# MrTornado24/IDE-3D

Hardware: AMD Instinct MI355X
Metric: 512x512 RGB+seg frames/s @96 depth samples (whole job) (higher is better)
Workload: dtype f32 (3x3 convs + MLPs: fp32 operands as 3 bf16 pieces, 6 products, f32 accumulate); 1 GPU; BASELINE config 2: random-init ide3d-ffhq-64-512, G.mapping + G.synthesis (64 render -> 512, 96 samples, RGB + 19-class seg) + uint8 frames, batch 4 seeds per GPU; global_batch=4, parallelism=dp1, conv_arithmetic=bf16x6, conv_arithmetic_is_library_default=True

## Files before the change

### ide-3d_amd/csrc/modconv.hip

```cpp
#include "common.h"
#include "knobs.h"
#include <stdlib.h>
#include <string.h>
#include <type_traits>

namespace ide3d {

typedef float f32x16 __attribute__((ext_vector_type(16)));

#ifdef IDE3D_MC_TRACE
__device__ unsigned long long g_mc_dbg[256];
#define IDE3D_MC_TS(k) { const unsigned long long now_ = __builtin_readcyclecounter(); mc_acc[k] += now_ - mc_last; mc_last = now_; }
#else
#define IDE3D_MC_TS(k)
#endif

enum { MODE_CONV3 = 0, MODE_CONV1 = 1, MODE_TCONV3 = 2, MODE_TCONV3A = 3, MODE_CONV3S2 = 4 };

template <int MODE> struct ModeCfg;
template <> struct ModeCfg<MODE_CONV3>  { static constexpr int KC = 4, WTAPS = 9, MAXT = 9; };
template <> struct ModeCfg<MODE_CONV1>  { static constexpr int KC = 16, WTAPS = 1, MAXT = 1; };
template <> struct ModeCfg<MODE_CONV3S2> { static constexpr int KC = 4, WTAPS = 9, MAXT = 9; };
template <> struct ModeCfg<MODE_TCONV3> { static constexpr int KC = 4, WTAPS = 9, MAXT = 4; };
template <> struct ModeCfg<MODE_TCONV3A> { static constexpr int KC = 4, WTAPS = 9, MAXT = 9; };

template <int MODE, int BIG, int TI, int PH, int PW>
struct McCfg {
    static constexpr int NWV = 4, NT = 64 * NWV;
    static constexpr int BN = TI * PH * PW;
    static_assert(BN == 64 || BN == 128 || BN == 256, "pixel tile must hold 64, 128 or 256 pixels");
    static constexpr int NCLS = (MODE == MODE_TCONV3A) ? 4 : 1;
    using MC = ModeCfg<MODE>;
    static constexpr int KC = MC::KC, WTAPS = MC::WTAPS, MAXT = MC::MAXT;
    static constexpr int WM = BIG ? 2 : 1, WN = NWV / WM;
    static constexpr int MTW = (BIG == 1) ? 2 : 1;
    static constexpr int NTW = (BN / 32) / WN;
    static constexpr int BM = WM * MTW * 32;
    static constexpr int STRIDE = (MODE == MODE_CONV3S2) ? 2 : 1;
    static constexpr int HALO = (MODE == MODE_CONV1 || MODE == MODE_CONV3S2) ? 0 : 1;
    static constexpr int HP = (MODE == MODE_CONV3S2) ? 2 * PH + 1 : PH + 2 * HALO;
    static constexpr int HW = (MODE == MODE_CONV3S2) ? 2 * PW + 1 : PW + 2 * HALO;
    static constexpr int XW = (MODE == MODE_CONV1) ? PW : (MODE == MODE_CONV3S2) ? ((HW + 3) & ~3) : ((PW == 16) ? 48 : HW + 2);
    static constexpr int XS = HP * XW;
    static constexpr int XI = KC * XS;
    static constexpr int LDS_W = MAXT * KC * BM;
    static constexpr int LDS_X = TI * XI;
    static constexpr int NW4 = (LDS_W / 4 + NT - 1) / NT;
    static constexpr int VW = (MODE == MODE_CONV1 && PH == 1 && PW % 4 == 0) ? 4 : 1;
    static constexpr int NXE = (TI * KC * HP * HW / VW + NT - 1) / NT;
};

template <int N>
__device__ __forceinline__ int sel(const int (&a)[N], int t) {
    int v = a[0];
#pragma unroll
    for (int i = 1; i < N; ++i) v = (t == i) ? a[i] : v;
    return v;
}

__host__ __device__ inline int mc_bm(int cout) { return cout > 96 ? 128 : (cout > 32 ? 64 : 32); }
__host__ __device__ inline int mc_kc(int k) { return k == 3 ? 4 : 16; }

__global__ void __launch_bounds__(256)
modconv_pack_kernel(const float* __restrict__ w, int64_t w_batch_stride, int nbatch, int cout, int cin, int taps, int bm, int kc,
                    int mblocks, int cchunks, float* __restrict__ out) {
    const int64_t total = (int64_t)nbatch * mblocks * cchunks * taps * kc * bm;
    const int64_t stride = (int64_t)gridDim.x * blockDim.x;
    for (int64_t i = (int64_t)blockIdx.x * blockDim.x + threadIdx.x; i < total; i += stride) {
        int64_t r = i;
        const int co_l = (int)(r % bm); r /= bm;
        const int cil = (int)(r % kc); r /= kc;
        const int tap = (int)(r % taps); r /= taps;
        const int cc = (int)(r % cchunks); r /= cchunks;
        const int mb = (int)(r % mblocks); r /= mblocks;
        const int nb = (int)r;
        const int co = mb * bm + co_l, ci = cc * kc + cil;
        out[i] = (co < cout && ci < cin) ? w[nb * w_batch_stride + ((int64_t)co * cin + ci) * taps + tap] : 0.f;
    }
}

struct ConvGeom {
    int tiles_x[4], tiles_y[4];
    int tile_base[5];
    int img_groups;
// ... 436 lines not shown
        const unsigned pk = pk_bf16(a, b);
        out[q] = pk;
        if (q + 1 < PARTS) { a -= __uint_as_float(pk << 16); b -= __uint_as_float(pk & 0xffff0000u); }
    }
    }
}
template <int F16>
__device__ __forceinline__ f32x16 sp_mfma(const u32x4& a, const u32x4& b, const f32x16& c) {
    if constexpr (F16) return __builtin_amdgcn_mfma_f32_32x32x16_f16(__builtin_bit_cast(f16x8, a), __builtin_bit_cast(f16x8, b), c, 0, 0, 0);
    else return __builtin_amdgcn_mfma_f32_32x32x16_bf16(__builtin_bit_cast(bf16x8, a), __builtin_bit_cast(bf16x8, b), c, 0, 0, 0);
}
__device__ __forceinline__ void f16_scale(float bound, float& scale, float& unscale) {
    scale = 1.f; unscale = 1.f;
    if (bound > 0.f && bound < __builtin_inff()) {
        int e;
        frexpf(bound, &e);
        e = min(max(15 - e, -126), 126);
        scale = ldexpf(1.f, e); unscale = ldexpf(1.f, -e);
    }
}

__global__ void __launch_bounds__(256)
modconv_row_scale_kernel(const float* __restrict__ w, int cout, int rowlen, int rows_padded, float* __restrict__ scale, float* __restrict__ unscale) {
    const int row = blockIdx.x * 4 + (threadIdx.x >> 6), lane = threadIdx.x & 63;
    if (row >= rows_padded) return;
    float m = 0.f;
    if (row < cout) for (int i = lane; i < rowlen; i += 64) m = fmaxf(m, fabsf(w[(int64_t)row * rowlen + i]));
#pragma unroll
    for (int off = 32; off > 0; off >>= 1) m = fmaxf(m, __shfl_xor(m, off));
    if (lane == 0) { float sc, us; f16_scale(m, sc, us); scale[row] = sc; unscale[row] = us; }
}

template <int PARTS, int F16 = 0>
__global__ void __launch_bounds__(256)
modconv_pack_split_kernel(const float* __restrict__ w, int cout, int cin, int bm, int mblocks, int cchunks, u32x4* __restrict__ out,
                          const float* __restrict__ row_scale = nullptr) {
    const int64_t total = (int64_t)mblocks * cchunks * 9 * 2 * bm;
    const int64_t stride = (int64_t)gridDim.x * blockDim.x;
    for (int64_t i = (int64_t)blockIdx.x * blockDim.x + threadIdx.x; i < total; i += stride) {
        int64_t r = i;
        const int co_l = (int)(r % bm); r /= bm;
        const int kg = (int)(r % 2); r /= 2;
        const int tap = (int)(r % 9); r /= 9;
        const int cc = (int)(r % cchunks); r /= cchunks;
        const int mb = (int)r;
        const int co = mb * bm + co_l;
        const float rs = F16 ? row_scale[co] : 1.f;
        unsigned pk[4][PARTS];
#pragma unroll
        for (int e = 0; e < 4; ++e) {
            const int ci = cc * 16 + kg * 8 + e * 2;
            const float a = (co < cout && ci < cin) ? w[((int64_t)co * cin + ci) * 9 + tap] * rs : 0.f;
            const float b = (co < cout && ci + 1 < cin) ? w[((int64_t)co * cin + ci + 1) * 9 + tap] * rs : 0.f;
            split_pair<PARTS, F16>(a, b, pk[e]);
        }
        const int64_t base = (((int64_t)(mb * cchunks + cc) * 9 + tap) * PARTS * 2 + kg) * bm + co_l;
#pragma unroll
        for (int q = 0; q < PARTS; ++q) {
            const u32x4 v = {pk[0][q], pk[1][q], pk[2][q], pk[3][q]};
            out[base + (int64_t)q * 2 * bm] = v;
        }
    }
}

template <int OFF_BYTES>
__device__ __forceinline__ u32x4 lds_read128_async(unsigned addr) {
    u32x4 v;
    asm volatile("ds_read_b128 %0, %1 offset:%2" : "=v"(v) : "v"(addr), "n"(OFF_BYTES));
    return v;
}
template <int PENDING>
__device__ __forceinline__ void lds_wait128(u32x4& first) { asm volatile("s_waitcnt lgkmcnt(%1)" : "+v"(first) : "n"(PENDING)); }
__device__ __forceinline__ void lds_pin128(u32x4& v) { asm volatile("" : "+v"(v)); }

struct HeadEpi {
    const u32x4* w;
    const float* bias;
    float* y;
    int rows;
    float clamp;
    int store_x;
    int bias_first;
};
template <int PH, int PW, int NWV, int MTW, int NTW, int BM, int MT, int PARTS, int SCRATCH>
__device__ __forceinline__ void split_heads_finish(const ide3d_modconv_params& p, const HeadEpi& he, f32x16 (&acc)[1][MTW][NTW], float* smem,
                                                   int n0, int y0, int x0, int wm, int wn, int lp) {
    constexpr int NT = 64 * NWV, BN = PH * PW, TP = BN + 4, ROWS = MT * 32, CCH = BM / 16, A_UNITS = PARTS * 2 * ROWS;
    static_assert(BM * TP + 2 * BM + ROWS <= SCRATCH, "activation tile + coefficients must fit the loop's LDS");
    const int tid = threadIdx.x, lane = tid & 63, half = lane >> 5, l32 = lane & 31;
    const int wid = __builtin_amdgcn_readfirstlane(tid >> 6);
    const int hw = p.h * p.w_;
    float* const s_t = smem;
    float* const s_dm = smem + BM * TP;
    float* const s_bi = s_dm + BM;
    float* const s_hb = s_bi + BM;
    for (int e = tid; e < BM; e += NT) {
        s_dm[e] = (p.dcoefs && e < p.cout) ? p.dcoefs[(int64_t)n0 * p.cout + e] : 1.f;
        s_bi[e] = (p.bias && e < p.cout) ? p.bias[e] : 0.f;
    }
    for (int e = tid; e < ROWS; e += NT) s_hb[e] = (he.bias && e < he.rows) ? he.bias[e] : 0.f;
    __syncthreads();
    const float e_alpha = (p.act == 3) ? p.alpha : 1.f, e_gain = p.gain;
    const float e_clamp = (p.clamp >= 0.f) ? p.clamp : __builtin_inff();
    const float e_nstr = p.noise ? p.noise_strength : 0.f;
    auto finish = [&](float v, float d, float nz, float bb) {
        v *= d; v += nz; v += bb;
        v = (v > 0.f) ? v : v * e_alpha;
        v *= e_gain;
        return fminf(fmaxf(v, -e_clamp), e_clamp);
    };
#pragma unroll
    for (int j = 0; j < NTW; ++j) {
        const int pix = (wn * NTW + j) * 32 + lp;
        const int gy = y0 + pix / PW, gx = x0 + pix % PW;
        const float nz = (e_nstr != 0.f) ? p.noise[gy * p.w_ + gx] * e_nstr : 0.f;
#pragma unroll
        for (int i = 0; i < MTW; ++i)
#pragma unroll
            for (int r = 0; r < 16; ++r) {
                const int rl = (wm * MTW + i) * 32 + (r & 3) + 8 * (r >> 2) + 4 * half;
                s_t[rl * TP + pix] = finish(acc[0][i][j][r], s_dm[rl], nz, s_bi[rl]);
            }
    }
    __syncthreads();
    typedef float f32x4a __attribute__((ext_vector_type(4)));
    typedef float f32x4u __attribute__((ext_vector_type(4), aligned(4)));
    if (he.store_x) {
        float* const yimg = p.y + (int64_t)n0 * p.cout * hw;
#pragma unroll 4
        for (int e = tid; e < BM * BN / 4; e += NT) {
            const int rl = e / (BN / 4), pix = (e % (BN / 4)) * 4;
            const int gy = y0 + pix / PW, gx = x0 + pix % PW;
            *reinterpret_cast<f32x4u*>(yimg + (int64_t)rl * hw + gy * p.w_ + gx) = *reinterpret_cast<const f32x4a*>(s_t + rl * TP + pix);
        }
    }
    constexpr int NPT = BN / 32;
    constexpr int RG = (MT % 2 == 0 && NPT / NWV < 2) ? 2 : 1, MTH = MT / RG, PG = NWV / RG, NTH = NPT / PG;
    static_assert(MTH * RG == MT && NTH * PG == NPT && NTH >= 1, "head work must split evenly over the waves");
    const int rg = wid / PG, pg = wid % PG;
    const u32x4* __restrict__ wsrc = he.w + (int64_t)n0 * CCH * A_UNITS + half * ROWS + rg * MTH * 32 + l32;
    f32x16 hacc[MTH][NTH];
#pragma unroll
    for (int m = 0; m < MTH; ++m)
#pragma unroll
        for (int g = 0; g < 4; ++g) {
            const f32x4a b4 = *reinterpret_cast<const f32x4a*>(s_hb + (rg * MTH + m) * 32 + 8 * g + 4 * half);
#pragma unroll
            for (int t = 0; t < NTH; ++t)
#pragma unroll
                for (int k = 0; k < 4; ++k) hacc[m][t][4 * g + k] = he.bias_first ? b4[k] : 0.f;
        }
    u32x4 af[2][MTH][PARTS];
    auto fetch_a = [&](int c, int buf) {
#pragma unroll
        for (int m = 0; m < MTH; ++m)
#pragma unroll
            for (int q = 0; q < PARTS; ++q) af[buf][m][q] = wsrc[(int64_t)c * A_UNITS + q * 2 * ROWS + m * 32];
    };
    fetch_a(0, 0);
#pragma unroll
    for (int c = 0; c < CCH; ++c) {
        const int ab = c & 1;
        if (c + 1 < CCH) fetch_a(c + 1, ab ^ 1);
#pragma unroll
        for (int t = 0; t < NTH; ++t) {
            const float* xs = s_t + (c * 16 + 8 * half) * TP + (pg * NTH + t) * 32 + l32;
            u32x4 bfrag[PARTS];
            {
                unsigned pk[4][PARTS];
#pragma unroll
                for (int e = 0; e < 4; ++e) split_pair<PARTS>(xs[(2 * e) * TP], xs[(2 * e + 1) * TP], pk[e]);
#pragma unroll
                for (int q = 0; q < PARTS; ++q) bfrag[q] = u32x4{pk[0][q], pk[1][q], pk[2][q], pk[3][q]};
            }
#pragma unroll
            for (int m = 0; m < MTH; ++m)
#pragma unroll
                for (int qa = 0; qa < PARTS; ++qa)
#pragma unroll
                    for (int qb = 0; qa + qb < PARTS; ++qb)
                        hacc[m][t] = __builtin_amdgcn_mfma_f32_32x32x16_bf16(__builtin_bit_cast(bf16x8, af[ab][m][qa]), __builtin_bit_cast(bf16x8, bfrag[qb]), hacc[m][t], 0, 0, 0);
        }
    }
    const float h_clamp = (he.clamp >= 0.f) ? he.clamp : __builtin_inff();
#pragma unroll
    for (int t = 0; t < NTH; ++t) {
        const int pix = (pg * NTH + t) * 32 + l32;
        const int gy = y0 + pix / PW, gx = x0 + pix % PW;
        float* const o = he.y + (int64_t)n0 * he.rows * hw + gy * p.w_ + gx;
#pragma unroll
        for (int m = 0; m < MTH; ++m)
#pragma unroll
            for (int r = 0; r < 16; ++r) {
                const int row = (rg * MTH + m) * 32 + 8 * (r >> 2) + 4 * half + (r & 3);
                if (row >= he.rows) continue;
                float v = hacc[m][t][r];
                if (he.bias_first) {
                    v = __builtin_amdgcn_fmed3f(v, -h_clamp, h_clamp);
                } else {
                    v *= 1.f; v += 0.f; v += s_hb[row];
                    v = (v > 0.f) ? v : v * 1.f;
                    v = fminf(fmaxf(v, -h_clamp), h_clamp);
                }
                o[(int64_t)row * hw] = v;
            }
    }
    __syncthreads();
}

template <int MODE, int BIG, int PH, int PARTS, int WBUF, int NWV, int F16, int TEAMS = 1, int PAR = -1, int HEAD_MT = 0>
__device__ __forceinline__ void modconv_split_tile(const ide3d_modconv_params& p, const u32x4* __restrict__ wp, float* __restrict__ partial,
                                                   const ConvGeom& g, unsigned char* smem, int mb, int tl, int grp, int split, int tiles_x,
                                                   const float* __restrict__ row_unscale, float* wg_scratch = nullptr, const HeadEpi* he = nullptr) {
    using K = SpCfg<MODE, BIG, PH, PARTS, WBUF, NWV, (PAR >= 0)>;
    static_assert(!F16 || PARTS == 2, "f16x3 = two fp16 pieces per operand");
    static_assert(PAR < 0 || (MODE == MODE_TCONV3A && WBUF == 2 && TEAMS == 1), "row-parity pairs: transposed form, two weight buffers, one team");
    constexpr int NST = (PAR < 0) ? 3 : (PAR == 0 ? 2 : 1);
    auto kys = [](int i) constexpr { return (PAR < 0) ? i : (PAR == 0 ? 2 * i : 1); };
    static_assert(TEAMS == 1 || (TEAMS == 2 && NWV == 4), "two teams of four waves, or one team");
    constexpr int PW = K::PW;
    const int tid = (TEAMS == 2) ? (int)(threadIdx.x & 255u) : (int)threadIdx.x, lane = tid & 63;
    const int wid = __builtin_amdgcn_readfirstlane(tid >> 6);
    const int wm = wid / K::WN, wn = wid % K::WN;
    const int half = lane >> 5, l32 = lane & 31;
    const int lp = ((((l32 >> 2) ^ (l32 >> 3) ^ (l32 >> 4)) & 1) << 4) | (l32 & 15);
    const int txi = tl % tiles_x, tyi = tl / tiles_x;
    const int y0 = tyi * PH, x0 = txi * PW;
    const int n0 = grp;
    u32x4* const s_w = reinterpret_cast<u32x4*>(smem);
    u32x4* const s_x = s_w + WBUF * K::W_UNITS;

    f32x16 acc[K::NCLS][K::MTW][K::NTW];
#pragma unroll
    for (int q = 0; q < K::NCLS; ++q)
#pragma unroll
        for (int i = 0; i < K::MTW; ++i)
#pragma unroll
            for (int j = 0; j < K::NTW; ++j)
#pragma unroll
                for (int r = 0; r < 16; ++r) acc[q][i][j][r] = 0.f;

    const int hw = p.h * p.w_;
    int x_src[K::NXR];
#pragma unroll
    for (int r = 0; r < K::NXR; ++r) {
        const int sidx = lane + 64 * r;
        const int ry = sidx / K::HW, rx = sidx % K::HW;
        const int yy = y0 - 1 + ry, xx = x0 - 1 + rx;
        x_src[r] = (sidx < K::NSLOT && yy >= 0 && yy < p.h && xx >= 0 && xx < p.w_) ? yy * p.w_ + xx : -1;
    }
    const float* __restrict__ ximg = p.x + (int64_t)n0 * p.cin * hw;
    float xreg[K::NXR][4];
    float sty[4];
    float xs = 1.f, xus = 1.f;
    if constexpr (F16) {
        float mm = p.styles ? 0.f : 1.f;
        if (p.styles) for (int ci = lane; ci < p.cin; ci += 64) mm = fmaxf(mm, fabsf(p.styles[(int64_t)n0 * p.cin + ci]));
        float xm = (lane < IDE3D_AMAX_SLOTS) ? p.x_amax[(int64_t)n0 * IDE3D_AMAX_FLOATS + lane * IDE3D_AMAX_STRIDE] : 0.f;
#pragma unroll
        for (int off = 32; off > 0; off >>= 1) { mm = fmaxf(mm, __shfl_xor(mm, off)); xm = fmaxf(xm, __shfl_xor(xm, off)); }
        f16_scale(mm * xm, xs, xus);
    }
    const bool stages_patch = (NWV == 4) || wid < 4;
    auto fetch_patch = [&](int c) {
        if (!stages_patch) return;
        const int ci0 = c * K::KC + wid * 4;
#pragma unroll
        for (int k = 0; k < 4; ++k) {
            const int ci = min(ci0 + k, p.cin - 1);
            sty[k] = (ci0 + k < p.cin) ? (p.styles ? p.styles[(int64_t)n0 * p.cin + ci] : 1.f) : 0.f;
#pragma unroll
            for (int r = 0; r < K::NXR; ++r) xreg[r][k] = ximg[(int64_t)ci * hw + max(x_src[r], 0)];
        }
    };
    auto commit_patch = [&](int buf) {
        if (!stages_patch) return;
        unsigned char* const dst = reinterpret_cast<unsigned char*>(s_x + buf * K::X_UNITS) + ((wid >> 1) * K::NSLOT) * 16 + (wid & 1) * 8;
        const float sc[4] = {F16 ? sty[0] * xs : sty[0], F16 ? sty[1] * xs : sty[1], F16 ? sty[2] * xs : sty[2], F16 ? sty[3] * xs : sty[3]};
#pragma unroll
        for (int r = 0; r < K::NXR; ++r) {
            const int sidx = lane + 64 * r;
            const bool live = x_src[r] >= 0;
            unsigned lo[PARTS], hi[PARTS];
            split_pair<PARTS, F16>(live ? xreg[r][0] * sc[0] : 0.f, live ? xreg[r][1] * sc[1] : 0.f, lo);
            split_pair<PARTS, F16>(live ? xreg[r][2] * sc[2] : 0.f, live ? xreg[r][3] * sc[3] : 0.f, hi);
            if (sidx < K::NSLOT) {
#pragma unroll
                for (int q = 0; q < PARTS; ++q) {
                    const u32x2 v = {lo[q], hi[q]};
                    *reinterpret_cast<u32x2*>(dst + (q * 2 * K::NSLOT + sidx) * 16) = v;
                }
            }
        }
    };
    const u32x4* __restrict__ wsrc = wp + (int64_t)mb * g.cchunks * 3 * K::W_UNITS;
    constexpr int W_PIECES = K::W_UNITS / 64;
// ... 44 lines not shown
        const bool more = c + 1 < c_end;
        static_for<NST>([&](auto sii) {
            constexpr int SI = decltype(sii)::value, KY = kys(SI);
            constexpr bool LAST = (SI == NST - 1), MID = (SI == (NST == 3 ? 1 : 0));
            const int next_stage = LAST ? (c + 1) * 3 + kys(0) : c * 3 + kys(LAST ? 0 : SI + 1);
            IDE3D_MC_TS(0)
            if constexpr (WBUF == 2) {
                if (!LAST || more) fetch_weights(next_stage, wbuf ^ 1);
                if (MID && more) fetch_patch(c + 1);
            } else {
                fetch_weights(c * 3 + KY, 0);
                if (MID && more) fetch_patch(c + 1);
                asm volatile("s_waitcnt vmcnt(0)" ::: "memory");
                __syncthreads();
            }
            IDE3D_MC_TS(1)
            const unsigned a_base = a_base0 + ((WBUF == 2) ? wbuf * (K::W_UNITS * 16) : 0);
            unsigned b_base[K::NTW];
#pragma unroll
            for (int j = 0; j < K::NTW; ++j) b_base[j] = b_base0[j] + xbuf * (K::X_UNITS * 16);
            constexpr int GRP = K::MTW + K::NTW, NGRP = 3 * PARTS;
            constexpr int SP_AHEAD = 1;
            constexpr int NBUF = (PARTS == 2 && SP_AHEAD > 1) ? 3 : 2;
            constexpr int AHEAD_CAP = 15 / GRP - 1, AHEAD_SAFE = (NBUF - 1) * PARTS - 1;
            constexpr int AHEAD = (SP_AHEAD < AHEAD_CAP ? SP_AHEAD : AHEAD_CAP) < AHEAD_SAFE ? (SP_AHEAD < AHEAD_CAP ? SP_AHEAD : AHEAD_CAP) : AHEAD_SAFE;
            static_assert(AHEAD >= 1 && (AHEAD + 1) * GRP <= 15, "lgkmcnt is a 4-bit counter");
            constexpr bool B_REUSE = (MODE == MODE_TCONV3A) && NBUF == 2;
            u32x4 av[NBUF][K::MTW][PARTS], bv[NBUF][K::NTW][PARTS];
            auto issue = [&](auto ss) {
                constexpr int S = decltype(ss)::value, KX = S / PARTS, Q = S % PARTS, B = KX % NBUF, T = KY * 3 + KX;
                constexpr int BS = B_REUSE ? (KX == 2 ? 1 : 0) : B;
                static_for<K::MTW>([&](auto ii) {
                    constexpr int I = decltype(ii)::value;
                    av[B][I][Q] = lds_read128_async<(((KX * PARTS + Q) * 2) * K::BM + I * 32) * 16>(a_base);
                });
                if constexpr (!(B_REUSE && KX == 1))
                static_for<K::NTW>([&](auto jj) {
                    constexpr int J = decltype(jj)::value;
                    bv[BS][J][Q] = lds_read128_async<(Q * 2 * K::NSLOT + tap_patch_offset<MODE, K::HW>(T)) * 16>(b_base[J]);
                });
            };
            static_for<AHEAD>([&](auto ss) { issue(ss); });
            static_for<NGRP>([&](auto ss) {
                constexpr int S = decltype(ss)::value, KX = S / PARTS, Q = S % PARTS, B = KX % NBUF, QC = (PAR >= 0) ? (KX & 1) : tap_class<MODE>(KY * 3 + KX);
                constexpr int BS = B_REUSE ? (KX == 2 ? 1 : 0) : B;
                if constexpr (S + AHEAD < NGRP) issue(std::integral_constant<int, S + AHEAD>{});
                constexpr int PENDING = [] { int n = 0; for (int s2 = S + 1; s2 <= S + AHEAD && s2 < NGRP; ++s2) n += K::MTW + ((B_REUSE && s2 / PARTS == 1) ? 0 : K::NTW); return n; }();
                lds_wait128<PENDING>(av[B][0][Q]);
#pragma unroll
                for (int i = 0; i < K::MTW; ++i) lds_pin128(av[B][i][Q]);
                if constexpr (!(B_REUSE && KX == 1)) {
#pragma unroll
                for (int j = 0; j < K::NTW; ++j) lds_pin128(bv[BS][j][Q]);
                }
#pragma unroll
                for (int qa = 0; qa <= Q; ++qa)
#pragma unroll
                    for (int qb = 0; qb <= Q; ++qb) {
                        if ((qa == Q || qb == Q) && qa + qb < PARTS) {
#pragma unroll
                            for (int i = 0; i < K::MTW; ++i)
#pragma unroll
                                for (int j = 0; j < K::NTW; ++j)
                                    acc[QC][i][j] = sp_mfma<F16>(av[B][i][qa], bv[BS][j][qb], acc[QC][i][j]);
                        }
                    }
            });
            IDE3D_MC_TS(2)
            if (LAST && more) commit_patch(xbuf ^ 1);
            if constexpr (WBUF == 2 && NWV == 8) { if (!LAST || more) fetch_weights(next_stage, wbuf ^ 1, true); }
            IDE3D_MC_TS(3)
            if (WBUF == 2) asm volatile("s_waitcnt vmcnt(0)" ::: "memory");
            IDE3D_MC_TS(4)
            __syncthreads();
            IDE3D_MC_TS(5)
            wbuf ^= 1;
        });
    }
#ifdef IDE3D_MC_TRACE
    const unsigned long long mc_t1 = __builtin_readcyclecounter();
#endif
    if constexpr (HEAD_MT > 0) {
        static_assert(MODE == MODE_CONV3 && TEAMS == 1 && !F16 && K::NCLS == 1, "fused heads: 3x3 split-bf16 layers");
        split_heads_finish<PH, PW, K::NWV, K::MTW, K::NTW, K::BM, HEAD_MT, PARTS, K::LDS_BYTES / 4>(p, *he, acc, reinterpret_cast<float*>(smem), n0, y0, x0, wm, wn, lp);
    } else
    modconv_finish<MODE, 1, PH, PW, K::NWV, K::NCLS, K::MTW, K::NTW, K::BM, K::LDS_BYTES / 4, PAR>(p, partial, g, acc, reinterpret_cast<float*>(smem), mb, n0, y0, x0, split, 0, wm, wn, lp,
                                                                                                F16 ? row_unscale : nullptr, xus, (TEAMS == 2) ? tid : -1, wg_scratch);
#ifdef IDE3D_MC_TRACE
    if (blockIdx.x == 100 && (threadIdx.x == 0 || threadIdx.x == 256)) {
        const int o = threadIdx.x ? 16 : 0;
        for (int k = 0; k < 6; ++k) g_mc_dbg[o + k] = mc_acc[k];
        g_mc_dbg[o + 7] = (unsigned long long)(c_end - c_begin) * 3;
        g_mc_dbg[o + 8] = mc_prologue;
        g_mc_dbg[o + 9] = __builtin_readcyclecounter() - mc_t1;
    }
#endif
}



constexpr int head_waves(int mt) { return mt == 1 ? 16 : 8; }
template <int PARTS, int MT>
struct HeadCfg {
    static constexpr int ROWS = MT * 32;
    static constexpr int A_UNITS = PARTS * 2 * ROWS;
    static constexpr int NWV = head_waves(MT);
    static constexpr int BN = 32 * NWV;
};
__host__ __device__ inline int64_t head_packed_units(int n, int cchunks, int parts, int mt) { return (int64_t)n * cchunks * parts * 2 * mt * 32; }

template <int PARTS>
__global__ void __launch_bounds__(256)
head_pack_split_kernel(const float* __restrict__ w, int64_t w_batch_stride, int n, int cout, int cin, int rows, int cchunks, u32x4* __restrict__ out) {
    const int64_t total = (int64_t)n * cchunks * 2 * rows;
    const int64_t stride = (int64_t)gridDim.x * blockDim.x;
    for (int64_t i = (int64_t)blockIdx.x * blockDim.x + threadIdx.x; i < total; i += stride) {
        int64_t r = i;
        const int row = (int)(r % rows); r /= rows;
        const int kg = (int)(r % 2); r /= 2;
        const int cc = (int)(r % cchunks); r /= cchunks;
        const int nb = (int)r;
        unsigned pk[4][PARTS];
#pragma unroll
        for (int e = 0; e < 4; ++e) {
            const int ci = cc * 16 + kg * 8 + e * 2;
            const float a = (row < cout && ci < cin) ? w[nb * w_batch_stride + (int64_t)row * cin + ci] : 0.f;
            const float b = (row < cout && ci + 1 < cin) ? w[nb * w_batch_stride + (int64_t)row * cin + ci + 1] : 0.f;
            split_pair<PARTS>(a, b, pk[e]);
        }
        const int64_t base = (((int64_t)nb * cchunks + cc) * PARTS * 2 + kg) * rows + row;
#pragma unroll
        for (int q = 0; q < PARTS; ++q) {
            const u32x4 v = {pk[0][q], pk[1][q], pk[2][q], pk[3][q]};
            out[base + (int64_t)q * 2 * rows] = v;
        }
    }
}

template <int PARTS, int MT>
__global__ void __launch_bounds__(64 * head_waves(MT), head_waves(MT) / 4)
head_split_kernel(ide3d_modconv_params p, const u32x4* __restrict__ wp, int cchunks, int tiles_per_image) {
    using K = HeadCfg<PARTS, MT>;
    if constexpr (K::NWV == 16) asm volatile("" ::: "v127"); else asm volatile("" ::: "v255");
    constexpr int S_MIN = K::NWV * 32 * 40 / 4 + 2 * K::ROWS / 4 + 16;
    constexpr int S_UNITS = (2 * K::A_UNITS > S_MIN) ? 2 * K::A_UNITS : S_MIN;
    __shared__ __attribute__((aligned(16))) u32x4 s_a[S_UNITS];
    const int tid = threadIdx.x, lane = tid & 63, half = lane >> 5, l32 = lane & 31;
    const int wid = __builtin_amdgcn_readfirstlane(tid >> 6);
    const int bid = xcd_remap(blockIdx.x, gridDim.x);
    const int n0 = bid / tiles_per_image, tile = bid % tiles_per_image;
    const int hw = p.h * p.w_;
    const int pix = tile * K::BN + wid * 32 + l32;
    const int pix_c = min(pix, hw - 1);
    const float* __restrict__ xl = p.x + (int64_t)n0 * p.cin * hw + (int64_t)(8 * half) * hw + pix_c;
    const u32x4* __restrict__ wsrc = wp + (int64_t)n0 * cchunks * K::A_UNITS;

    f32x16 acc[1][MT][1];
#pragma unroll
    for (int m = 0; m < MT; ++m)
#pragma unroll
        for (int r = 0; r < 16; ++r) acc[0][m][0][r] = 0.f;

    constexpr int A_PIECES = K::A_UNITS / 64;
    static_assert(K::A_UNITS % 64 == 0, "whole 1 KB pieces");
    auto fetch_a = [&](int c, int buf) {
        for (int i = wid; i < A_PIECES; i += K::NWV)
            __builtin_amdgcn_global_load_lds((const __attribute__((address_space(1))) void*)(wsrc + (int64_t)c * K::A_UNITS + i * 64 + lane),
// ... 321 lines not shown
                const float vb = ok_b ? xb[k] * scv[k] : 0.f;
                const float4 a0 = wv[0], a1 = wv[1], c0v = wv[4], c1v = wv[5];
                const float w0[STRIP_CO] = {a0.x, a0.y, a0.z, a0.w, a1.x, a1.y, a1.z, a1.w};
                const float w2[STRIP_CO] = {c0v.x, c0v.y, c0v.z, c0v.w, c1v.x, c1v.y, c1v.z, c1v.w};
#pragma unroll
                for (int j = 0; j < STRIP_CO; ++j) { acc[j] = fmaf(va, w0[j], acc[j]); acc[j] = fmaf(vb, w2[j], acc[j]); }
            }
        }
    }
#pragma unroll
    for (int j = 0; j < STRIP_CO; ++j) s_red[q][j][lane] = acc[j];
    __syncthreads();
    float am = 0.f;
    {
        static_assert(STRIP_CO <= STRIP_WAVES, "wave q < STRIP_CO finishes output channel co0 + q");
        float v = 0.f;
        const int qc = min(q, STRIP_CO - 1);
#pragma unroll
        for (int k = 0; k < STRIP_WAVES; ++k) v += s_red[k][qc][lane];
        const int co = co0 + q;
        if (live && q < STRIP_CO && co < p.cout) {
            v *= p.dcoefs ? p.dcoefs[(int64_t)n * p.cout + co] : 1.f;
            const int oy = is_row ? oh - 1 : t, ox = is_row ? t : ow - 1;
            p.y[((int64_t)n * p.cout + co) * ((int64_t)oh * pitch) + (int64_t)oy * pitch + ox] = v;
            amax_acc(am, v);
        }
    }
    if (p.y_amax) amax_raise_block(p.y_amax, n, am, s_am);
}

struct BlockId { int mb, tile, grp, split; };
__device__ __forceinline__ BlockId decode_block(const ConvGeom& g) {
    int bid = xcd_remap(blockIdx.x, gridDim.x);
    BlockId b;
    b.mb = bid % g.mblocks; bid /= g.mblocks;
    b.tile = bid % g.tile_base[4]; bid /= g.tile_base[4];
    b.grp = bid % g.img_groups; bid /= g.img_groups;
    b.split = bid;
    return b;
}

template <int MODE, int BIG, int TI, int PH, int PW>
__global__ void __launch_bounds__(256, (McCfg<MODE, BIG, TI, PH, PW>::NCLS * McCfg<MODE, BIG, TI, PH, PW>::MTW * McCfg<MODE, BIG, TI, PH, PW>::NTW > 8) ? 1
                                       : (TI * PH * PW <= 128 && MODE != MODE_CONV3S2) ? 3 : 2)
modconv_kernel(ide3d_modconv_params p, const float* __restrict__ wp, float* __restrict__ partial, ConvGeom g) {
    using K = McCfg<MODE, BIG, TI, PH, PW>;
    __shared__ __attribute__((aligned(16))) float s_w[2 * K::LDS_W];
    __shared__ __attribute__((aligned(16))) float s_x[2 * K::LDS_X];
    const BlockId b = decode_block(g);
    int cls = 0;
    if (MODE == MODE_TCONV3) { cls = (b.tile >= g.tile_base[1]) + (b.tile >= g.tile_base[2]) + (b.tile >= g.tile_base[3]); }
    modconv_tile<MODE, BIG, TI, PH, PW>(p, wp, partial, g, s_w, s_x, b.mb, b.tile - g.tile_base[cls], b.grp, b.split, cls, g.tiles_x[cls]);
}


#ifdef IDE3D_SP_SHARED_SIMD
constexpr bool kSpExclusive = false;
#else
constexpr bool kSpExclusive = true;
#endif
template <int MODE, int BIG, int PH, int PARTS, int WBUF, int NWV>
constexpr int sp_waves_per_simd() {
    using K = SpCfg<MODE, BIG, PH, PARTS, WBUF, NWV>;
    return (NWV == 8) ? 2 : (!kSpExclusive && K::LDS_BYTES <= 80 * 1024 && (WBUF == 1 || K::NCLS * K::MTW * K::NTW <= 8)) ? 2 : 1;
}
template <int MODE, int BIG, int PH, int PARTS, int WBUF = 2, int NWV = 4, int F16 = 0>
__global__ void __launch_bounds__(64 * NWV, (sp_waves_per_simd<MODE, BIG, PH, PARTS, WBUF, NWV>()))
modconv_split_kernel(ide3d_modconv_params p, const u32x4* __restrict__ wp, float* __restrict__ partial, ConvGeom g, const float* __restrict__ row_unscale) {
    using K = SpCfg<MODE, BIG, PH, PARTS, WBUF, NWV>;
    if constexpr (kSpExclusive) { if constexpr (NWV == 8) asm volatile("" ::: "v255"); else asm volatile("" ::: "v255", "a255"); }
    __shared__ __attribute__((aligned(16))) unsigned char sp_smem[K::LDS_BYTES];
    const BlockId b = decode_block(g);
    modconv_split_tile<MODE, BIG, PH, PARTS, WBUF, NWV, F16>(p, wp, partial, g, sp_smem, b.mb, b.tile, b.grp, b.split, g.tiles_x[0], row_unscale);
}

template <int BIG, int PH, int HEAD_MT>
__global__ void __launch_bounds__(512, 2)
modconv_split_heads_kernel(ide3d_modconv_params p, const u32x4* __restrict__ wp, ConvGeom g, HeadEpi he) {
    using K = SpCfg<MODE_CONV3, BIG, PH, 3, 2, 8>;
    if constexpr (kSpExclusive) asm volatile("" ::: "v255");
    __shared__ __attribute__((aligned(16))) unsigned char sp_smem[K::LDS_BYTES];
    const BlockId b = decode_block(g);
    modconv_split_tile<MODE_CONV3, BIG, PH, 3, 2, 8, 0, 1, -1, HEAD_MT>(p, wp, nullptr, g, sp_smem, b.mb, b.tile, b.grp, b.split, g.tiles_x[0], nullptr, nullptr, &he);
}

template <int BIG, int PH, int PARTS, int F16 = 0>
__global__ void __launch_bounds__(512, 2)
modconv_split_pair_kernel(ide3d_modconv_params p, const u32x4* __restrict__ wp, float* __restrict__ partial, ConvGeom g, const float* __restrict__ row_unscale) {
    using K = SpCfg<MODE_TCONV3A, BIG, PH, PARTS, 2, 8, 1>;
    if constexpr (kSpExclusive) asm volatile("" ::: "v255");
    __shared__ __attribute__((aligned(16))) unsigned char sp_smem[K::LDS_BYTES];
    const int half_grid = (int)(gridDim.x >> 1);
    const int par = __builtin_amdgcn_readfirstlane((int)blockIdx.x >= half_grid ? 1 : 0);
    int bid = xcd_remap((int)blockIdx.x - par * half_grid, half_grid);
    BlockId b;
    b.mb = bid % g.mblocks; bid /= g.mblocks;
    b.tile = bid % g.tile_base[4]; bid /= g.tile_base[4];
    b.grp = bid % g.img_groups; bid /= g.img_groups;
    b.split = bid;
    if (par == 0) modconv_split_tile<MODE_TCONV3A, BIG, PH, PARTS, 2, 8, F16, 1, 0>(p, wp, partial, g, sp_smem, b.mb, b.tile, b.grp, b.split, g.tiles_x[0], row_unscale);
    else          modconv_split_tile<MODE_TCONV3A, BIG, PH, PARTS, 2, 8, F16, 1, 1>(p, wp, partial, g, sp_smem, b.mb, b.tile, b.grp, b.split, g.tiles_x[0], row_unscale);
}

template <int MODE, int BIG, int PH, int PARTS, int WBUF, int F16>
__global__ void __launch_bounds__(512, 2)
modconv_split_teams_kernel(ide3d_modconv_params p, const u32x4* __restrict__ wp, float* __restrict__ partial, ConvGeom g, const float* __restrict__ row_unscale) {
    using K = SpCfg<MODE, BIG, PH, PARTS, WBUF, 4>;
    static_assert(2 * K::LDS_BYTES <= 160 * 1024, "both teams' LDS must fit");
    asm volatile("" ::: "v255");
    __shared__ __attribute__((aligned(16))) unsigned char sp_smem[2 * K::LDS_BYTES];
    const int team = (int)(threadIdx.x >> 8);
    int bid = xcd_remap(blockIdx.x, gridDim.x);
    const int mpairs = g.mblocks >> 1;
    BlockId b;
    b.mb = 2 * (bid % mpairs) + team; bid /= mpairs;
    b.tile = bid % g.tile_base[4]; bid /= g.tile_base[4];
    b.grp = bid % g.img_groups; bid /= g.img_groups;
    b.split = bid;
    modconv_split_tile<MODE, BIG, PH, PARTS, WBUF, 4, F16, 2>(p, wp, partial, g, sp_smem + team * K::LDS_BYTES, b.mb, b.tile, b.grp, b.split, g.tiles_x[0], row_unscale,
                                                              reinterpret_cast<float*>(sp_smem));
}

__global__ void __launch_bounds__(256)
modconv_epilogue_kernel(ide3d_modconv_params p, const float* __restrict__ partial, int split_k, int oh, int ow) {
    const int64_t per = (int64_t)p.n * p.cout * oh * ow;
    const int64_t stride = (int64_t)gridDim.x * blockDim.x;
    int am_n = -1; float am = 0.f;
    __shared__ unsigned s_am[64];
    const bool am_lds = p.y_amax && p.n <= 64;
    if (p.y_amax) { if (threadIdx.x < 64) s_am[threadIdx.x] = 0u; __syncthreads(); }
    const int hw = oh * ow;
    if (p.y_pitch <= 0 && (hw & 3) == 0) {
        typedef float f32x4v __attribute__((ext_vector_type(4)));
        const int64_t per4 = per >> 2;
        for (int64_t q = (int64_t)blockIdx.x * blockDim.x + threadIdx.x; q < per4; q += stride) {
            const int64_t i = q << 2;
            f32x4v v = {0.f, 0.f, 0.f, 0.f};
            int s = 0;
            for (; s + 4 <= split_k; s += 4) {
                f32x4v t[4];
#pragma unroll
                for (int k = 0; k < 4; ++k) t[k] = *reinterpret_cast<const f32x4v*>(partial + (int64_t)(s + k) * per + i);
#pragma unroll
                for (int k = 0; k < 4; ++k) v += t[k];
            }
            for (; s < split_k; ++s) v += *reinterpret_cast<const f32x4v*>(partial + (int64_t)s * per + i);
            const int pix = (int)(i % hw);
            const int co = (int)((i / hw) % p.cout);
            const int n = (int)(i / ((int64_t)hw * p.cout));
            const float d = p.dcoefs ? p.dcoefs[(int64_t)n * p.cout + co] : 1.f, bb = p.bias ? p.bias[co] : 0.f;
#pragma unroll
            for (int e = 0; e < 4; ++e) {
                float x = v[e];
                if (p.dcoefs) x *= d;
                if (p.noise) x += p.noise[pix + e] * p.noise_strength;
                if (p.bias) x += bb;
                if (p.act == 3) x = (x > 0.f) ? x : x * p.alpha;
                x *= p.gain;
                if (p.clamp >= 0.f) x = fminf(fmaxf(x, -p.clamp), p.clamp);
                v[e] = x;
            }
            *reinterpret_cast<f32x4v*>(p.y + i) = v;
            if (p.y_amax) {
                if (n != am_n) { if (am_n >= 0) { if (am_lds) amax_lds_flush(s_am, am_n, am); else amax_commit(p.y_amax, am_n, am, false); } am_n = n; am = 0.f; }
                amax_acc(am, v[0]); amax_acc(am, v[1]); amax_acc(am, v[2]); amax_acc(am, v[3]);
            }
// ... 361 lines not shown
    IDE3D_CHECK_ARG(p.act == 1 || p.act == 3, "modconv2d: act must be linear (1) or lrelu (3)");
    IDE3D_CHECK_ARG(p.y_pitch == 0 || (p.mode == 2 && p.y_pitch >= 2 * p.w_ + 1), "modconv2d: y_pitch is the row pitch of a transposed convolution's output (>= 2 w + 1), or 0");
    hipStream_t st_head = (hipStream_t)stream;
    {
        const int64_t hw = (int64_t)p.h * p.w_;
        if (head_small_applies(p)) {
            if (hw <= 64) hipLaunchKernelGGL((head_small_kernel<64, 32>), dim3(cdiv(p.cout, HS_RB), 1, p.n), dim3(HS_THREADS), 0, st_head, p, (int)hw);
            else          hipLaunchKernelGGL((head_small_kernel<256, 8>), dim3(cdiv(p.cout, HS_RB), cdiv((int)hw, 256), p.n), dim3(HS_THREADS), 0, st_head, p, (int)hw);
            IDE3D_CHECK_LAUNCH("modconv2d (small-map heads)");
            return IDE3D_OK;
        }
    }
    if (head_split_applies(p, resolve_arith(p.arith))) {
        const int parts = resolve_arith(p.arith) == 3 ? 2 : 3, mt = p.cout <= 32 ? 1 : 6, cchunks = cdiv(p.cin, 16);
        IDE3D_CHECK_ARG(p.workspace_bytes >= head_packed_units(p.n, cchunks, parts, mt) * 16, "modconv2d: workspace too small for the packed head weights");
        u32x4* wu = reinterpret_cast<u32x4*>(p.workspace);
        const int64_t items = (int64_t)p.n * cchunks * 2 * mt * 32;
        const int tiles = cdiv(p.h * p.w_, 32 * head_waves(mt));
        const int hw_h = p.h * p.w_, wgs_img = kNumCU / p.n, tiles32 = hw_h / 32;
        const bool resident = head_resident_applies(p);
#define IDE3D_HEAD_RES(P, M, C) IDE3D_EXCL_LAUNCH((head_resident_kernel<P, M, C>), dim3(p.n * wgs_img), 512, 0, st_head, p, wu, wgs_img, tiles32)
#define IDE3D_HEAD(P, M) do { \
            hipLaunchKernelGGL(head_pack_split_kernel<P>, dim3(stream_grid(items, 256)), dim3(256), 0, st_head, p.w, p.w_batch_stride, p.n, p.cout, p.cin, M * 32, cchunks, wu); \
            if (resident) { if (M == 6) IDE3D_HEAD_RES(P, 6, 8); else if (cchunks == 4) IDE3D_HEAD_RES(P, 1, 4); else IDE3D_HEAD_RES(P, 1, 8); } \
            else IDE3D_EXCL_LAUNCH((head_split_kernel<P, M>), dim3(p.n * tiles), 64 * head_waves(M), 0, st_head, p, wu, cchunks, tiles); } while (0)
        if (parts == 2) { if (mt == 1) IDE3D_HEAD(2, 1); else IDE3D_HEAD(2, 6); }
        else            { if (mt == 1) IDE3D_HEAD(3, 1); else IDE3D_HEAD(3, 6); }
#undef IDE3D_HEAD
#undef IDE3D_HEAD_RES
        IDE3D_CHECK_LAUNCH("modconv2d (split-bf16 heads)");
        return IDE3D_OK;
    }
    int arith_eff = resolve_arith(p.arith);
    if (arith_eff == 16 && !p.x_amax) arith_eff = 6;
    ConvPlan pl; plan_conv(p, pl, arith_eff);
    IDE3D_CHECK_ARG(p.workspace_bytes >= (pl.packed_floats + pl.aux_floats + pl.partial_floats) * (int64_t)sizeof(float),
                    "modconv2d: workspace too small (need %lld bytes)", (long long)((pl.packed_floats + pl.aux_floats + pl.partial_floats) * sizeof(float)));
    hipStream_t st = (hipStream_t)stream;
    float* wp = p.workspace;
    float* partial = p.workspace + pl.packed_floats + pl.aux_floats;
    if (pl.parts) {
        if (!p.weights_packed) pack_split_weights(p, pl, wp, st);
#define IDE3D_SP_DISPATCH(M) \
        do { if (pl.big == 1) { if (pl.f16) launch_split<M, 1, 2, 1>(p, pl, wp, partial, st); else if (pl.parts == 2) launch_split<M, 1, 2>(p, pl, wp, partial, st); else launch_split<M, 1, 3>(p, pl, wp, partial, st); } \
             else             { if (pl.f16) launch_split<M, 2, 2, 1>(p, pl, wp, partial, st); else if (pl.parts == 2) launch_split<M, 2, 2>(p, pl, wp, partial, st); else launch_split<M, 2, 3>(p, pl, wp, partial, st); } } while (0)
        if (pl.mode == MODE_CONV3) IDE3D_SP_DISPATCH(MODE_CONV3); else IDE3D_SP_DISPATCH(MODE_TCONV3A);
#undef IDE3D_SP_DISPATCH
    } else {
    if (!p.weights_packed) {
        hipLaunchKernelGGL(modconv_pack_kernel, dim3(stream_grid(pl.packed_floats, 256)), dim3(256), 0, st,
                           p.w, p.w_batch_stride, p.w_batch_stride ? p.n : 1, p.cout, p.cin, pl.taps, pl.bm, pl.kc, pl.mblocks, pl.cchunks, wp);
    }
#define IDE3D_MC_DISPATCH(M) \
    do { if (pl.big == 1) launch_tiles<M, 1>(p, pl, wp, partial, st); else if (pl.big == 2) launch_tiles<M, 2>(p, pl, wp, partial, st); \
         else launch_tiles<M, 0>(p, pl, wp, partial, st); } while (0)
    if (pl.mode == MODE_CONV3)       IDE3D_MC_DISPATCH(MODE_CONV3);
    else if (pl.mode == MODE_CONV1)  IDE3D_MC_DISPATCH(MODE_CONV1);
    else if (pl.mode == MODE_CONV3S2) IDE3D_MC_DISPATCH(MODE_CONV3S2);
    else if (pl.mode == MODE_TCONV3A) IDE3D_MC_DISPATCH(MODE_TCONV3A);
    else                             IDE3D_MC_DISPATCH(MODE_TCONV3);
#undef IDE3D_MC_DISPATCH
    }
    if (pl.g.split_k > 1) {
        const int64_t per = (int64_t)p.n * p.cout * pl.oh * pl.ow;
        hipLaunchKernelGGL(modconv_epilogue_kernel, dim3(stream_grid((p.y_pitch <= 0 && ((pl.oh * pl.ow) & 3) == 0) ? per / 4 : per, 256)), dim3(256), 0, st, p, partial, pl.g.split_k, pl.oh, pl.ow);
    }
    if (pl.mode == MODE_TCONV3A && !p.weights_packed) {
        hipLaunchKernelGGL(tconv_strip_pack_kernel, dim3(stream_grid(pl.strip_floats, 256)), dim3(256), 0, st, p.w, p.cout, p.cin, cdiv(p.cout, STRIP_CO) * STRIP_CO,
                           wp + pl.packed_floats + pl.strip_off);
    }
    if (pl.strip) {
        const int cout_pad = cdiv(p.cout, STRIP_CO) * STRIP_CO;
        float* const wstrip = wp + pl.packed_floats + pl.strip_off;
        const int nb_re = cdiv(p.w_ + 1, 64), nb_ro = cdiv(p.w_, 64), nb_ce = cdiv(p.h, 64), nb_co = cdiv(p.h, 64);
        float* const xs = wstrip + pl.strip_floats;
        hipLaunchKernelGGL(tconv_strip_gather_kernel, dim3(stream_grid((int64_t)p.n * p.cin * (p.h + p.w_), 256)), dim3(256), 0, st, p.x, p.n * p.cin, p.h, p.w_, xs);
        hipLaunchKernelGGL(tconv_strip_kernel, dim3(nb_re + nb_ro + nb_ce + nb_co, cout_pad / STRIP_CO, p.n), dim3(64 * STRIP_WAVES), 0, st, p, wstrip, xs, cout_pad,
                           pl.oh, pl.ow, (int64_t)(p.y_pitch > 0 ? p.y_pitch : pl.ow), nb_re, nb_ro, nb_ce);
    }
    IDE3D_CHECK_LAUNCH("modconv2d");
    return IDE3D_OK;
}

extern "C" int ide3d_modconv2d_heads(const ide3d_modconv_params* pp, const ide3d_modconv_head_epilogue* hp, void* stream) {
    using namespace ide3d;
    IDE3D_CHECK_ARG(pp != nullptr && hp != nullptr, "modconv2d_heads: null params");
    const ide3d_modconv_params& p = *pp;
    const ide3d_modconv_head_epilogue& h = *hp;
    IDE3D_CHECK_ARG(p.x && p.w && p.workspace && (p.y || h.no_activation_output) && h.w && h.y && h.workspace, "modconv2d_heads: null tensor / workspace pointer");
    int rc = check_modconv(p);
    if (rc) return rc;
    IDE3D_CHECK_ARG(p.act == 1 || p.act == 3, "modconv2d_heads: act must be linear (1) or lrelu (3)");
    IDE3D_CHECK_ARG(h.rows > 0, "modconv2d_heads: bad head rows");
    auto no_kernel = [](const char* why) { set_error("modconv2d_heads: %s", why); return IDE3D_ENOKERNEL; };
    if (knob_live("IDE3D_MODCONV_NO_HEAD_FUSION")) return no_kernel("IDE3D_MODCONV_NO_HEAD_FUSION is set");
    if (p.k != 3 || p.mode != 0 || p.w_batch_stride != 0 || p.y_amax || p.y_pitch != 0) return no_kernel("not a shared-weight 3x3 layer without side outputs");
    int arith = resolve_arith(p.arith);
    if (arith == 16 && !p.x_amax) arith = 6;
    if (arith != 6) return no_kernel("the fused form exists for bf16x6 only");
    ConvPlan pl; plan_conv(p, pl, arith);
    if (pl.parts != 3 || pl.f16 || pl.mode != MODE_CONV3 || pl.pair || pl.g.split_k != 1 || pl.g.mblocks != 1 || pl.bm != p.cout || kTiles[pl.tile].images != 1)
        return no_kernel("the layer's plan does not hold all channels of a tile in one workgroup");
    const bool tile16 = pl.big == 1 && p.cout == 128 && pl.tile == T16x16 && sp_form(pl).waves == 8;
    const bool tile32 = pl.big == 2 && p.cout == 64 && pl.tile == T32x16;
    const int ph = tile32 ? 32 : 16;
    if (!(tile16 || tile32) || p.h % ph != 0 || p.w_ % 16 != 0) return no_kernel("no fused instance for this tile");
    ide3d_modconv_params q{};
    q.x = p.y; q.w = h.w; q.bias = h.bias; q.y = h.y;
    q.n = p.n; q.cin = p.cout; q.cout = h.rows; q.h = p.h; q.w_ = p.w_; q.k = 1; q.mode = 0;
    q.act = 1; q.alpha = 0.f; q.gain = 1.f; q.clamp = h.clamp; q.w_batch_stride = (int64_t)h.rows * p.cout; q.arith = p.arith;
    const int mt = h.rows <= 32 ? 1 : 6, hcc = p.cout / 16;
    if (head_small_applies(q) || !head_split_applies(q, resolve_arith(q.arith)) || resolve_arith(q.arith) == 3 || (mt == 6 && !tile16))
        return no_kernel("the heads do not take the split-bf16 path");
    IDE3D_CHECK_ARG(p.workspace_bytes >= (pl.packed_floats + pl.aux_floats) * (int64_t)sizeof(float), "modconv2d_heads: workspace too small");
    IDE3D_CHECK_ARG(h.workspace_bytes >= head_packed_units(p.n, hcc, 3, mt) * 16, "modconv2d_heads: head workspace too small");
    hipStream_t st = (hipStream_t)stream;
    if (!p.weights_packed) pack_split_weights(p, pl, p.workspace, st);
    u32x4* const hw_packed = reinterpret_cast<u32x4*>(h.workspace);
    const int64_t items = (int64_t)p.n * hcc * 2 * mt * 32;
    hipLaunchKernelGGL(head_pack_split_kernel<3>, dim3(stream_grid(items, 256)), dim3(256), 0, st, h.w, q.w_batch_stride, p.n, h.rows, p.cout, mt * 32, hcc, hw_packed);
    HeadEpi e;
    e.w = hw_packed; e.bias = h.bias; e.y = h.y; e.rows = h.rows; e.clamp = h.clamp; e.store_x = !h.no_activation_output;
    e.bias_first = head_resident_applies(q) ? 1 : 0;
    const ConvGeom& g = pl.g;
    const unsigned nblocks = (unsigned)((int64_t)g.mblocks * g.tile_base[4] * g.img_groups * g.split_k);
    const u32x4* wu = reinterpret_cast<const u32x4*>(p.workspace);
    if (tile32) IDE3D_EXCL_LAUNCH((modconv_split_heads_kernel<2, 32, 1>), dim3(nblocks), 512, 0, st, p, wu, g, e);
    else if (mt == 1) IDE3D_EXCL_LAUNCH((modconv_split_heads_kernel<1, 16, 1>), dim3(nblocks), 512, 0, st, p, wu, g, e);
    else IDE3D_EXCL_LAUNCH((modconv_split_heads_kernel<1, 16, 6>), dim3(nblocks), 512, 0, st, p, wu, g, e);
    IDE3D_CHECK_LAUNCH("modconv2d_heads");
    return IDE3D_OK;
}

extern "C" int ide3d_modconv_plan(const ide3d_modconv_params* pp, ide3d_modconv_plan_info* out) {
    using namespace ide3d;
    IDE3D_CHECK_ARG(pp != nullptr && out != nullptr, "modconv_plan: null argument");
    const ide3d_modconv_params p = flatten_pointwise(*pp);
    int rc = check_modconv(p);
    if (rc) return rc;
    *out = ide3d_modconv_plan_info{};
    const int arith = resolve_arith(p.arith);
    if (head_small_applies(p)) {
        const int hw = p.h * p.w_;
        out->kind = IDE3D_PLAN_HEAD_SMALL; out->tile_h = 1; out->tile_w = hw <= 64 ? 64 : 256; out->rows = HS_RB; out->waves = HS_THREADS / 64; out->split_k = 1;
        out->workgroups = (int64_t)cdiv(p.cout, HS_RB) * (hw <= 64 ? 1 : cdiv(hw, 256)) * p.n;
        return IDE3D_OK;
    }
    if (head_split_applies(p, arith)) {
        const int mt = p.cout <= 32 ? 1 : 6;
        out->rows = mt * 32; out->parts = arith == 3 ? 2 : 3; out->split_k = 1; out->tile_h = 1;
        if (head_resident_applies(p)) { out->kind = IDE3D_PLAN_HEAD_RESIDENT; out->tile_w = 32; out->waves = 8; out->workgroups = (int64_t)p.n * (kNumCU / p.n); }
        else { out->kind = IDE3D_PLAN_HEAD_SPLIT; out->waves = head_waves(mt); out->tile_w = 32 * out->waves; out->workgroups = (int64_t)p.n * cdiv(p.h * p.w_, out->tile_w); }
        return IDE3D_OK;
    }
    int arith_eff = arith;
    if (arith_eff == 16 && !p.x_amax) arith_eff = 6;
    ConvPlan pl; plan_conv(p, pl, arith_eff);
    const int64_t blocks = (int64_t)pl.g.mblocks * pl.g.tile_base[4] * pl.g.img_groups * pl.g.split_k * (pl.pair ? 2 : 1);
    out->tile_h = kTiles[pl.tile].rows; out->tile_w = kTiles[pl.tile].cols; out->images_per_tile = kTiles[pl.tile].images;
    out->rows = pl.bm; out->parts = pl.parts; out->f16 = pl.f16; out->split_k = pl.g.split_k; out->strip = pl.strip;
    out->transposed_all_class = (pl.mode == MODE_TCONV3A);
    if (pl.parts) {
        const SpForm f = sp_form(pl);
        out->kind = f.teams ? IDE3D_PLAN_SPLIT_TEAMS : IDE3D_PLAN_SPLIT; out->waves = f.teams ? 8 : f.waves; out->workgroups = f.teams ? blocks / 2 : blocks;
    } else {
        out->kind = IDE3D_PLAN_FP32; out->waves = 4; out->workgroups = blocks;
    }
    return IDE3D_OK;
}

extern "C" int ide3d_set_conv_arithmetic(int32_t arith) {
    IDE3D_CHECK_ARG(arith == 0 || arith == 1 || arith == 3 || arith == 6 || arith == 16,
                    "set_conv_arithmetic: 0 (environment default), 1 (fp32), 3 (bf16x3), 6 (bf16x6) or 16 (f16x3)");
    ide3d::g_conv_arith = arith;
    return IDE3D_OK;
}
extern "C" int32_t ide3d_get_conv_arithmetic(void) { return ide3d::conv_arith_default(); }

#ifdef IDE3D_MC_TRACE
extern "C" int ide3d_debug_mc(unsigned long long* host) {
    return (int)hipMemcpyFromSymbol(host, HIP_SYMBOL(ide3d::g_mc_dbg), sizeof(unsigned long long) * 256);
}
#endif

namespace ide3d {
const char* modconv_build_flags() {
    return ""
#ifdef IDE3D_SP_SHARED_SIMD
        "!IDE3D_SP_SHARED_SIMD "
#endif
#ifdef IDE3D_MC_TRACE
        "IDE3D_MC_TRACE "
#endif
        ;
}
}
```

### ide-3d_amd/csrc/resample.hip

```cpp
#include "common.h"

namespace ide3d {
namespace {

constexpr int SK_ROWS = 8, SK_COLS = 32, SK_CH = 32;
constexpr int SK_LR = SK_ROWS / 2 + 2, SK_LC = SK_COLS / 2 + 2;
constexpr int SK_TP = SK_CH + 1;

struct SkipArgs {
    const float* lo; const float* add; float* out;
    int64_t lo_s[4], add_s[4];
    int n, c, h, w;
    int tiles_x, tiles_y, cgroups;
};

__global__ void __launch_bounds__(256)
skip_upsample_add_cl_kernel(const SkipArgs p) {
    __shared__ float s_lo[SK_CH][SK_LR][SK_LC + 1];
    __shared__ float s_t[SK_ROWS * SK_COLS][SK_TP];
    const int tid = threadIdx.x;
    int b = xcd_remap(blockIdx.x, gridDim.x);
    const int cg = b % p.cgroups; b /= p.cgroups;
    const int tx = b % p.tiles_x; b /= p.tiles_x;
    const int ty = b % p.tiles_y; b /= p.tiles_y;
    const int n = b;
    const int c0 = cg * SK_CH, Y0 = ty * SK_ROWS, X0 = tx * SK_COLS;
    const int H = 2 * p.h, W = 2 * p.w;
    const int m0 = Y0 / 2 - 1, q0 = X0 / 2 - 1;
    constexpr int NLO = (SK_CH * SK_LR * SK_LC + 255) / 256;
    float lo_v[NLO];
#pragma unroll
    for (int i = 0; i < NLO; ++i) {
        const int e = tid + i * 256;
        const int c = e / (SK_LR * SK_LC), r = e % (SK_LR * SK_LC), ry = r / SK_LC, rx = r % SK_LC;
        const int yy = m0 + ry, xx = q0 + rx;
        const bool ok = e < SK_CH * SK_LR * SK_LC && c0 + c < p.c && yy >= 0 && yy < p.h && xx >= 0 && xx < p.w;
        const int64_t off = n * p.lo_s[0] + (int64_t)min(c0 + c, p.c - 1) * p.lo_s[1] + (int64_t)min(max(yy, 0), p.h - 1) * p.lo_s[2]
                          + (int64_t)min(max(xx, 0), p.w - 1) * p.lo_s[3];
        const float v = p.lo[off];
        lo_v[i] = ok ? v : 0.f;
    }
    const int row = tid >> 5, x = tid & 31;
    const int Y = Y0 + row, X = X0 + x;
    const bool ok = Y < H && X < W;
    float add_v[SK_CH];
    {
        const float* ap = p.add + n * p.add_s[0] + (int64_t)min(Y, H - 1) * p.add_s[2] + (int64_t)min(X, W - 1) * p.add_s[3];
#pragma unroll
        for (int c = 0; c < SK_CH; ++c) add_v[c] = ap[(int64_t)min(c0 + c, p.c - 1) * p.add_s[1]];
    }
#pragma unroll
    for (int i = 0; i < NLO; ++i) {
        const int e = tid + i * 256;
        if (e < SK_CH * SK_LR * SK_LC) {
            const int c = e / (SK_LR * SK_LC), r = e % (SK_LR * SK_LC);
            s_lo[c][r / SK_LC][r % SK_LC] = lo_v[i];
        }
    }
    __syncthreads();
    {
        const int ly = (Y >> 1) - m0 - 1 + (Y & 1), lx = (X >> 1) - q0 - 1 + (X & 1);
        const float wy0 = (Y & 1) ? 0.75f : 0.25f, wy1 = 1.0f - wy0;
        const float wx0 = (X & 1) ? 0.75f : 0.25f, wx1 = 1.0f - wx0;
#pragma unroll
        for (int c = 0; c < SK_CH; ++c) {
            const float a = s_lo[c][ly][lx], bq = s_lo[c][ly][lx + 1], cq = s_lo[c][ly + 1][lx], d = s_lo[c][ly + 1][lx + 1];
            float v = wy0 * (wx0 * a + wx1 * bq) + wy1 * (wx0 * cq + wx1 * d);
            if (ok && c0 + c < p.c) v += add_v[c];
            s_t[tid][c] = v;
        }
    }
    __syncthreads();
    {
        const int j = tid & 7;
#pragma unroll
        for (int k = 0; k < 8; ++k) {
            const int px = (tid >> 3) + 32 * k, row = px >> 5, x = px & 31;
            const int Y = Y0 + row, X = X0 + x;
            if (Y >= H || X >= W) continue;
            float* o = p.out + (((int64_t)n * H + Y) * W + X) * p.c + c0 + 4 * j;
            const float* t = &s_t[px][4 * j];
            if (c0 + 4 * j + 3 < p.c) {
                typedef float f32x4_t __attribute__((ext_vector_type(4)));
                const f32x4_t v = {t[0], t[1], t[2], t[3]};
                __builtin_nontemporal_store(v, reinterpret_cast<f32x4_t*>(o));
            } else {
                for (int e = 0; e < 4; ++e) if (c0 + 4 * j + e < p.c) o[e] = t[e];
            }
        }
    }
}

struct BilinArgs {
    const float* x; int n, c, h, w;
    float* dst[3]; int c_begin[3], c_count[3];
    int64_t bs[3];
};

__global__ void __launch_bounds__(256)
bilinear_up2_split_kernel(const BilinArgs p) {
    const int H = 2 * p.h, W = 2 * p.w, W4 = W / 4;
    const int ctot = p.c_count[0] + p.c_count[1] + p.c_count[2];
    const int64_t total = (int64_t)p.n * ctot * H * W4;
    const int64_t stride = (int64_t)gridDim.x * blockDim.x;
    for (int64_t i = (int64_t)blockIdx.x * blockDim.x + threadIdx.x; i < total; i += stride) {
        int64_t r = i;
        const int X = (int)(r % W4) * 4; r /= W4;
        const int Y = (int)(r % H); r /= H;
        int cc = (int)(r % ctot);
        const int n = (int)(r / ctot);
        int k = 0;
        if (cc >= p.c_count[0]) { cc -= p.c_count[0]; k = 1; if (cc >= p.c_count[1]) { cc -= p.c_count[1]; k = 2; } }
        const int ci = p.c_begin[k] + cc;
        const float sy = fmaxf(0.5f * ((float)Y + 0.5f) - 0.5f, 0.f);
        const int y0 = (int)sy, y1 = y0 + (y0 < p.h - 1);
        const float ly1 = sy - (float)y0, ly0 = 1.f - ly1;
        const float* r0 = p.x + ((int64_t)n * p.c + ci) * ((int64_t)p.h * p.w) + (int64_t)y0 * p.w;
        const float* r1 = r0 + (int64_t)(y1 - y0) * p.w;
        float o[4];
#pragma unroll
        for (int e = 0; e < 4; ++e) {
            const float sx = fmaxf(0.5f * ((float)(X + e) + 0.5f) - 0.5f, 0.f);
            const int x0 = (int)sx, x1 = x0 + (x0 < p.w - 1);
            const float lx1 = sx - (float)x0, lx0 = 1.f - lx1;
            o[e] = ly0 * (lx0 * r0[x0] + lx1 * r0[x1]) + ly1 * (lx0 * r1[x0] + lx1 * r1[x1]);
        }
        *reinterpret_cast<float4*>(p.dst[k] + (int64_t)n * p.bs[k] + ((int64_t)cc * H + Y) * W + X) = make_float4(o[0], o[1], o[2], o[3]);
    }
}

}
}

extern "C" int ide3d_skip_upsample_add_cl(const float* lo, const int64_t lo_stride[4], const float* add, const int64_t add_stride[4],
                                          int32_t n, int32_t c, int32_t h, int32_t w, float* out, void* stream) {
    using namespace ide3d;
    IDE3D_CHECK_ARG(lo && add && out && lo_stride && add_stride, "skip_upsample_add_cl: null pointer");
    IDE3D_CHECK_ARG(n > 0 && c > 0 && h > 0 && w > 0, "skip_upsample_add_cl: bad shape");
    IDE3D_CHECK_ARG(c % 4 == 0 && (reinterpret_cast<uintptr_t>(out) & 15) == 0, "skip_upsample_add_cl: channels must be a multiple of 4 and out 16-byte aligned");
    SkipArgs a;
    a.lo = lo; a.add = add; a.out = out;
    for (int i = 0; i < 4; ++i) { a.lo_s[i] = lo_stride[i]; a.add_s[i] = add_stride[i]; }
    a.n = n; a.c = c; a.h = h; a.w = w;
    a.tiles_x = cdiv(2 * w, SK_COLS); a.tiles_y = cdiv(2 * h, SK_ROWS); a.cgroups = cdiv(c, SK_CH);
    const int64_t blocks = (int64_t)n * a.tiles_x * a.tiles_y * a.cgroups;
    IDE3D_CHECK_ARG(blocks < 0x7fffffffLL, "skip_upsample_add_cl: too many tiles");
    hipLaunchKernelGGL(skip_upsample_add_cl_kernel, dim3((unsigned)blocks), dim3(256), 0, (hipStream_t)stream, a);
    IDE3D_CHECK_LAUNCH("skip_upsample_add_cl");
    return IDE3D_OK;
}
// ... 26 lines not shown
```

### ide-3d_amd/csrc/upfirdn2d.hip

```cpp
#include "common.h"
#include "knobs.h"
#include <type_traits>

namespace ide3d {

template <class T>
__device__ __forceinline__ typename Elem<T>::math_t
apply_epilogue(typename Elem<T>::math_t v, const ide3d_upfirdn2d_epilogue& ep, int n, int c, int oy, int ox, int out_w) {
    using M = typename Elem<T>::math_t;
    if (ep.add) v += Elem<T>::ld((const T*)ep.add + n * ep.add_stride[0] + c * ep.add_stride[1] + oy * ep.add_stride[2] + ox * ep.add_stride[3]);
    if (ep.noise) v += (M)(ep.noise[oy * out_w + ox] * ep.noise_strength);
    if (ep.fused_act) {
        if (ep.bias) v += Elem<T>::ld((const T*)ep.bias + c);
        if (ep.act == 3) v = (v > 0) ? v : v * (M)ep.alpha;
        v *= (M)ep.act_gain;
        if (ep.clamp >= 0.f) v = (v > (M)ep.clamp) ? (M)ep.clamp : ((v < -(M)ep.clamp) ? -(M)ep.clamp : v);
    }
    return v;
}

template <class T, int NO>
__device__ __forceinline__ void epilogue_row(typename Elem<T>::math_t (&row)[NO], const ide3d_upfirdn2d_epilogue& ep,
                                             const T* add_plane, typename Elem<T>::math_t bias, int oy, int ox0, int out_w, bool full) {
    using M = typename Elem<T>::math_t;
    if (ep.add) {
        const T* ap = add_plane + (int64_t)oy * ep.add_stride[2];
        if constexpr (sizeof(T) == 4 && NO == 4) {
            if (full && ep.add_stride[3] == 1 && ((reinterpret_cast<uintptr_t>(ap + ox0) & 15) == 0)) {
                const float4 a = *reinterpret_cast<const float4*>(ap + ox0);
                row[0] += a.x; row[1] += a.y; row[2] += a.z; row[3] += a.w;
                goto add_done;
            }
        }
#pragma unroll
        for (int j = 0; j < NO; ++j) {
            const int ox = ox0 + j;
            if (ox >= 0 && ox < out_w) row[j] += Elem<T>::ld(ap + (int64_t)ox * ep.add_stride[3]);
        }
    }
add_done:
    if (ep.noise) {
        const float* np_ = ep.noise + (int64_t)oy * out_w;
        if (NO == 4 && full && ((reinterpret_cast<uintptr_t>(np_ + ox0) & 15) == 0)) {
            const float4 a = *reinterpret_cast<const float4*>(np_ + ox0);
            row[0] += (M)(a.x * ep.noise_strength); row[1] += (M)(a.y * ep.noise_strength);
            row[2] += (M)(a.z * ep.noise_strength); row[3] += (M)(a.w * ep.noise_strength);
        } else {
#pragma unroll
            for (int j = 0; j < NO; ++j) {
                const int ox = ox0 + j;
                if (ox >= 0 && ox < out_w) row[j] += (M)(np_[ox] * ep.noise_strength);
            }
        }
    }
    if (ep.fused_act) {
#pragma unroll
        for (int j = 0; j < NO; ++j) {
            M v = row[j] + bias;
            if (ep.act == 3) v = (v > 0) ? v : v * (M)ep.alpha;
            v *= (M)ep.act_gain;
            if (ep.clamp >= 0.f) v = (v > (M)ep.clamp) ? (M)ep.clamp : ((v < -(M)ep.clamp) ? -(M)ep.clamp : v);
            row[j] = v;
        }
    }
}


template <class T>
__global__ void __launch_bounds__(256)
upfirdn2d_generic_kernel(ide3d_upfirdn2d_params p, ide3d_upfirdn2d_epilogue ep, int c_fastest) {
    using M = typename Elem<T>::math_t;
    const T* __restrict__ x = (const T*)p.x;
    T* __restrict__ y = (T*)p.y;
    const int64_t total = (int64_t)p.n * p.c * p.out_h * p.out_w;
    const int64_t stride = (int64_t)gridDim.x * blockDim.x;
    int am_n = -1; float am = 0.f;
    __shared__ unsigned s_am[64];
    const bool am_lds = ep.y_amax && p.n <= 64;
    if (ep.y_amax) { if (threadIdx.x < 64) s_am[threadIdx.x] = 0u; __syncthreads(); }
    for (int64_t idx = (int64_t)blockIdx.x * blockDim.x + threadIdx.x; idx < total; idx += stride) {
        int ox, oy, c, n;
        int64_t r = idx;
        if (c_fastest) {
            c = (int)(r % p.c); r /= p.c;
// ... 413 lines not shown
__global__ void __launch_bounds__(256)
fir_up2_kernel(ide3d_upfirdn2d_params p, ide3d_upfirdn2d_epilogue ep, int tiles_x, int tiles_y) {
    using AX = Axis<2, 1, 4>;
    constexpr int TCX = 64, TCY = 16, LW = 72, LH = TCY + 2, NV = LW / 4, NLD = (LH * NV + 255) / 256;
    static_assert(AX::window(TCX) + 3 <= LW && AX::NT == 2 && AX::window(2) == 4, "window of the 4-tap polyphase filter");
    __shared__ __attribute__((aligned(16))) float s_in[LH * LW];
    float g[4][4];
#pragma unroll
    for (int ky = 0; ky < 4; ++ky)
#pragma unroll
        for (int kx = 0; kx < 4; ++kx) {
            const int fy = p.flip ? ky : 3 - ky, fx = p.flip ? kx : 3 - kx;
            g[ky][kx] = p.f[fy * p.f_stride[0] + fx * p.f_stride[1]] * p.gain;
        }
    int bid = xcd_remap(blockIdx.x, gridDim.x);
    const int tx_i = bid % tiles_x; bid /= tiles_x;
    const int ty_i = bid % tiles_y; bid /= tiles_y;
    const int n = bid / p.c, c = bid % p.c;
    const int qx0 = floordiv(-p.pad_x0, 2) + tx_i * TCX, qy0 = floordiv(-p.pad_y0, 2) + ty_i * TCY;
    const int x_al = qx0 & ~3, xoff = qx0 - x_al;
    const float* __restrict__ xp = (const float*)p.x + n * p.x_stride[0] + c * p.x_stride[1];
    const unsigned pitch = (unsigned)p.x_stride[2];
    const int w4 = (p.in_w + 3) & ~3;
    {
        float4 v4[NLD];
        int gy[NLD], gx[NLD];
#pragma unroll
        for (int k = 0; k < NLD; ++k) {
            const int idx = (int)threadIdx.x + k * 256;
            const int ly = idx / NV, lv = idx - ly * NV;
            gy[k] = qy0 + ly; gx[k] = x_al + 4 * lv;
            const unsigned cy_ = (unsigned)min(max(gy[k], 0), p.in_h - 1), cx_ = (unsigned)min(max(gx[k], 0), w4 - 4);
            v4[k] = *reinterpret_cast<const float4*>(xp + (cy_ * pitch + cx_));
        }
#pragma unroll
        for (int k = 0; k < NLD; ++k) {
            const int idx = (int)threadIdx.x + k * 256;
            if (idx < LH * NV) {
                const bool rowok = (unsigned)gy[k] < (unsigned)p.in_h;
                float4 w = v4[k];
                w.x = (rowok && (unsigned)(gx[k] + 0) < (unsigned)p.in_w) ? w.x : 0.f;
                w.y = (rowok && (unsigned)(gx[k] + 1) < (unsigned)p.in_w) ? w.y : 0.f;
                w.z = (rowok && (unsigned)(gx[k] + 2) < (unsigned)p.in_w) ? w.z : 0.f;
                w.w = (rowok && (unsigned)(gx[k] + 3) < (unsigned)p.in_w) ? w.w : 0.f;
                *reinterpret_cast<float4*>(s_in + 4 * idx) = w;
            }
        }
    }
    __syncthreads();
    const int tx = threadIdx.x & 31, ty = threadIdx.x >> 5;
    float win[4][4];
    {
        const float* wsrc = s_in + (ty * 2) * LW + tx * 2 + xoff;
#pragma unroll
        for (int wy = 0; wy < 4; ++wy)
#pragma unroll
            for (int wx = 0; wx < 4; ++wx) win[wy][wx] = wsrc[wy * LW + wx];
    }
    const bool has_add = ep.add != nullptr, has_noise = ep.noise != nullptr, act_on = ep.fused_act != 0;
    const float nstr = ep.noise_strength;
    const float bias = (act_on && ep.bias) ? ((const float*)ep.bias)[c] : 0.f;
    const bool lrelu = act_on && ep.act == 3, lrelu_max = lrelu && ep.alpha >= 0.f && ep.alpha <= 1.f;
    const float alpha = ep.alpha, again = act_on ? ep.act_gain : 1.f;
    const bool clamp_on = act_on && ep.clamp >= 0.f;
    const float cl = ep.clamp;
    float* __restrict__ yp = (float*)p.y + n * p.y_stride[0] + c * p.y_stride[1];
    const float* __restrict__ ap = has_add ? (const float*)ep.add + n * ep.add_stride[0] + c * ep.add_stride[1] : nullptr;
    const unsigned ypitch = (unsigned)p.y_stride[2], apitch = (unsigned)ep.add_stride[2];
    const int ox0 = (qx0 + tx * 2) * 2 + p.pad_x0;
    const bool full = ox0 >= 0 && ox0 + 4 <= p.out_w;
    float amax_t = 0.f;
    if (full) {
#pragma unroll
        for (int cy = 0; cy < 2; ++cy)
#pragma unroll
            for (int ry = 0; ry < 2; ++ry) {
                const int oy = (qy0 + ty * 2 + cy) * 2 + ry + p.pad_y0;
                if (oy < 0 || oy >= p.out_h) continue;
                float row[4];
#pragma unroll
                for (int cx = 0; cx < 2; ++cx)
#pragma unroll
                    for (int rx = 0; rx < 2; ++rx) {
                        float acc = 0.f;
#pragma unroll
                        for (int ty_ = 0; ty_ < 2; ++ty_)
#pragma unroll
                            for (int tx_ = 0; tx_ < 2; ++tx_)
                                acc += win[cy + AX::off(ry) + ty_][cx + AX::off(rx) + tx_] * g[AX::first(ry) + ty_ * 2][AX::first(rx) + tx_ * 2];
                        row[cx * 2 + rx] = acc;
                    }
                if (has_add) {
                    const float4 a = *reinterpret_cast<const float4*>(ap + ((unsigned)oy * apitch + (unsigned)ox0));
                    row[0] += a.x; row[1] += a.y; row[2] += a.z; row[3] += a.w;
                }
                if (has_noise) {
                    const float4 a = *reinterpret_cast<const float4*>(ep.noise + ((unsigned)oy * (unsigned)p.out_w + (unsigned)ox0));
                    row[0] += a.x * nstr; row[1] += a.y * nstr; row[2] += a.z * nstr; row[3] += a.w * nstr;
                }
                if (act_on) {
#pragma unroll
                    for (int j = 0; j < 4; ++j) {
                        float v = row[j] + bias;
                        if (lrelu_max) v = fmaxf(v, v * alpha);
                        else if (lrelu) v = (v > 0.f) ? v : v * alpha;
                        v *= again;
                        if (clamp_on) v = (v > cl) ? cl : ((v < -cl) ? -cl : v);
                        row[j] = v;
                    }
                }
#pragma unroll
                for (int j = 0; j < 4; ++j) amax_t = fmaxf(amax_t, fabsf(row[j]));
                *reinterpret_cast<float4*>(yp + ((unsigned)oy * ypitch + (unsigned)ox0)) = make_float4(row[0], row[1], row[2], row[3]);
            }
    }
    if (ep.y_amax) amax_raise_block(ep.y_amax, n, amax_t, s_in);
}

static bool fir_up2_applies(const ide3d_upfirdn2d_params& p, const ide3d_upfirdn2d_epilogue& ep) {
    const bool off = knob_live("IDE3D_FIR_NO_LEAN");
    if (off || p.dtype != IDE3D_F32 || p.f_w != 4 || p.f_h != 4 || p.up_x != 2 || p.up_y != 2 || p.down_x != 1 || p.down_y != 1) return false;
    if (p.x_stride[3] != 1 || p.y_stride[3] != 1 || (p.out_w & 3) || (p.in_w & 3)) return false;
    if (p.pad_x0 & 1) return false;
    const int64_t pitch = p.x_stride[2];
    if ((pitch & 3) || pitch < p.in_w || pitch <= 0 || p.y_stride[2] <= 0) return false;
    if ((reinterpret_cast<uintptr_t>(p.x) & 15) || (p.x_stride[0] & 3) || (p.x_stride[1] & 3)) return false;
    if ((reinterpret_cast<uintptr_t>(p.y) & 15) || (p.y_stride[0] & 3) || (p.y_stride[1] & 3) || (p.y_stride[2] & 3)) return false;
    if (ep.add && (ep.add_stride[3] != 1 || (reinterpret_cast<uintptr_t>(ep.add) & 15) || (ep.add_stride[0] & 3) || (ep.add_stride[1] & 3) || (ep.add_stride[2] & 3) ||
                   ep.add_stride[2] <= 0 || ep.add_stride[2] * (int64_t)p.out_h >= (1ll << 29))) return false;
    if (ep.noise && (reinterpret_cast<uintptr_t>(ep.noise) & 15)) return false;
    if (pitch * p.in_h >= (1ll << 29) || p.y_stride[2] * (int64_t)p.out_h >= (1ll << 29) || (int64_t)p.out_w * p.out_h >= (1ll << 29)) return false;
    return true;
}

static int launch_fir_up2(const ide3d_upfirdn2d_params& p, const ide3d_upfirdn2d_epilogue& ep, hipStream_t st) {
    auto cells = [](int out, int pad0) { return floordiv(out - 1 - pad0, 2) - floordiv(-pad0, 2) + 1; };
    const int tiles_x = cdiv(cells(p.out_w, p.pad_x0), 64), tiles_y = cdiv(cells(p.out_h, p.pad_y0), 16);
    const int64_t nblocks = (int64_t)tiles_x * tiles_y * p.n * p.c;
    if (nblocks > 0x7fffffff) { set_error("upfirdn2d: grid too large"); return IDE3D_EINVAL; }
    hipLaunchKernelGGL(fir_up2_kernel, dim3((unsigned)nblocks), dim3(256), 0, st, p, ep, tiles_x, tiles_y);
    IDE3D_CHECK_LAUNCH("upfirdn2d (fir_up2)");
    return IDE3D_OK;
}

template <class T, int UX, int UY, int DX, int DY, int FW, int FH, int CX, int CY>
static int launch_tile(const ide3d_upfirdn2d_params& p, const ide3d_upfirdn2d_epilogue& ep, hipStream_t st) {
    constexpr int TCX = 32 * CX, TCY = 8 * CY;
    auto cells = [](int out, int pad0, int U) {
        if (U == 1) return out;
        const int q_min = floordiv(-pad0, U);
        const int q_max = floordiv(out - 1 - pad0, U);
        return q_max - q_min + 1;
    };
    const int tiles_x = cdiv(cells(p.out_w, p.pad_x0, UX), TCX);
    const int tiles_y = cdiv(cells(p.out_h, p.pad_y0, UY), TCY);
    const int64_t nblocks = (int64_t)tiles_x * tiles_y * p.n * p.c;
    if (nblocks > 0x7fffffff) { set_error("upfirdn2d: grid too large"); return IDE3D_EINVAL; }
    hipLaunchKernelGGL((upfirdn2d_tile_kernel<T, UX, UY, DX, DY, FW, FH, CX, CY>), dim3((unsigned)nblocks),
                       dim3(256), 0, st, p, ep, tiles_x, tiles_y);
    IDE3D_CHECK_LAUNCH("upfirdn2d_tile");
    return IDE3D_OK;
}

template <class T>
static int launch_generic(const ide3d_upfirdn2d_params& p, const ide3d_upfirdn2d_epilogue& ep, hipStream_t st) {
    const int64_t total = (int64_t)p.n * p.c * p.out_h * p.out_w;
    const int c_fastest = (p.y_stride[1] == 1 && p.c > 1) ? 1 : 0;
    hipLaunchKernelGGL((upfirdn2d_generic_kernel<T>), dim3(stream_grid(total, 256)), dim3(256), 0, st, p, ep, c_fastest);
    IDE3D_CHECK_LAUNCH("upfirdn2d_generic");
    return IDE3D_OK;
}

template <class T, int U>
// ... 88 lines not shown
```

### ide-3d_amd/torch_utils/hip_plugin.py

```python

import ctypes
import math
import os
import threading
import weakref

import torch

_LIB_ENV = 'IDE3D_HIP_LIB'
_ABI_VERSION = 8
AMAX_SLOTS, AMAX_STRIDE = 32, 64
AMAX_FLOATS = AMAX_SLOTS * AMAX_STRIDE

_DTYPE_CODE = {torch.float32: 0, torch.float16: 1, torch.bfloat16: 2, torch.float64: 3}

_lock = threading.Lock()
_lib = None

CALLS = {}


def lib_path():
    env = os.environ.get(_LIB_ENV)
    if env:
# ... 57 lines not shown


class _RenderGrads(ctypes.Structure):
    _fields_ = [
        ('grad_feat', ctypes.c_void_p), ('grad_depth', ctypes.c_void_p), ('grad_wsum', ctypes.c_void_p),
        ('grad_tex_planes', ctypes.c_void_p), ('grad_geo_planes', ctypes.c_void_p),
        ('grad_tex_stride', ctypes.c_int64 * 4), ('grad_geo_stride', ctypes.c_int64 * 4),
    ]


class _RenderParamGrads(ctypes.Structure):
    _fields_ = [
        ('grad_geo_w0', ctypes.c_void_p), ('grad_geo_b0', ctypes.c_void_p), ('grad_geo_w1', ctypes.c_void_p), ('grad_geo_b1', ctypes.c_void_p),
        ('grad_tex_w0', ctypes.c_void_p), ('grad_tex_b0', ctypes.c_void_p), ('grad_tex_w1', ctypes.c_void_p), ('grad_tex_b1', ctypes.c_void_p),
        ('workspace', ctypes.c_void_p), ('workspace_bytes', ctypes.c_int64),
    ]


class _RenderCameraGrads(ctypes.Structure):
    _fields_ = [('grad_cam2world', ctypes.c_void_p), ('workspace', ctypes.c_void_p), ('workspace_bytes', ctypes.c_int64)]


class _Lattice(ctypes.Structure):
    _fields_ = [('n', ctypes.c_int32), ('voxel_size', ctypes.c_float), ('corner', ctypes.c_float * 3), ('scale', ctypes.c_float)]


class _RenderParams(ctypes.Structure):
    _fields_ = [
        ('rays_d_cam', ctypes.c_void_p), ('z_lin', ctypes.c_void_p), ('cam2world', ctypes.c_void_p),
        ('jitter', ctypes.c_void_p), ('sigma_noise', ctypes.c_void_p),
        ('tex_planes', ctypes.c_void_p), ('geo_planes', ctypes.c_void_p),
        ('tex_stride', ctypes.c_int64 * 4), ('geo_stride', ctypes.c_int64 * 4),
        ('geo_w0', ctypes.c_void_p), ('geo_b0', ctypes.c_void_p), ('geo_w1', ctypes.c_void_p), ('geo_b1', ctypes.c_void_p),
        ('tex_w0', ctypes.c_void_p), ('tex_b0', ctypes.c_void_p), ('tex_w1', ctypes.c_void_p), ('tex_b1', ctypes.c_void_p),
        ('n', ctypes.c_int32), ('rays_per_img', ctypes.c_int32), ('steps', ctypes.c_int32),
        ('C', ctypes.c_int32), ('H', ctypes.c_int32), ('W', ctypes.c_int32),
        ('hidden', ctypes.c_int32), ('feat_ch', ctypes.c_int32), ('seg_ch', ctypes.c_int32),
        ('clamp_mode', ctypes.c_int32), ('last_back', ctypes.c_int32), ('white_back', ctypes.c_int32),
        ('max_depth', ctypes.c_float),
        ('out_feat', ctypes.c_void_p), ('out_depth', ctypes.c_void_p), ('out_wsum', ctypes.c_void_p),
    ]


class _ModconvParams(ctypes.Structure):
    _fields_ = [
        ('x', ctypes.c_void_p), ('w', ctypes.c_void_p), ('styles', ctypes.c_void_p), ('dcoefs', ctypes.c_void_p),
        ('noise', ctypes.c_void_p), ('bias', ctypes.c_void_p), ('y', ctypes.c_void_p),
        ('n', ctypes.c_int32), ('cin', ctypes.c_int32), ('cout', ctypes.c_int32),
        ('h', ctypes.c_int32), ('w_', ctypes.c_int32), ('k', ctypes.c_int32),
        ('noise_strength', ctypes.c_float),
        ('act', ctypes.c_int32), ('alpha', ctypes.c_float), ('gain', ctypes.c_float), ('clamp', ctypes.c_float),
        ('mode', ctypes.c_int32), ('weights_packed', ctypes.c_int32),
        ('workspace', ctypes.c_void_p), ('workspace_bytes', ctypes.c_int64),
        ('w_batch_stride', ctypes.c_int64), ('arith', ctypes.c_int32),
        ('x_amax', ctypes.c_void_p), ('y_amax', ctypes.c_void_p), ('y_pitch', ctypes.c_int32),
    ]


class _ActBwdParams(ctypes.Structure):
    _fields_ = [
        ('dy', ctypes.c_void_p), ('y', ctypes.c_void_p), ('dz', ctypes.c_void_p),
        ('noise', ctypes.c_void_p), ('noise_strength', ctypes.c_float), ('bias', ctypes.c_void_p),
        ('dcoefs', ctypes.c_void_p), ('ddcoefs', ctypes.c_void_p),
        ('n', ctypes.c_int32), ('c', ctypes.c_int32), ('h', ctypes.c_int32), ('w', ctypes.c_int32), ('y_pitch', ctypes.c_int32),
        ('act', ctypes.c_int32), ('alpha', ctypes.c_float), ('gain', ctypes.c_float), ('clamp', ctypes.c_float),
        ('workspace', ctypes.c_void_p), ('workspace_bytes', ctypes.c_int64),
    ]


class _WgradParams(ctypes.Structure):
    _fields_ = [
        ('g', ctypes.c_void_p), ('x', ctypes.c_void_p), ('styles', ctypes.c_void_p), ('dcoefs', ctypes.c_void_p), ('dw', ctypes.c_void_p),
        ('n', ctypes.c_int32), ('cin', ctypes.c_int32), ('cout', ctypes.c_int32), ('h', ctypes.c_int32), ('w', ctypes.c_int32),
        ('mode', ctypes.c_int32), ('arith', ctypes.c_int32), ('workspace', ctypes.c_void_p), ('workspace_bytes', ctypes.c_int64),
    ]


class _ModconvHeadEpilogue(ctypes.Structure):
    _fields_ = [
        ('w', ctypes.c_void_p), ('bias', ctypes.c_void_p), ('y', ctypes.c_void_p),
        ('rows', ctypes.c_int32), ('clamp', ctypes.c_float), ('no_activation_output', ctypes.c_int32),
        ('workspace', ctypes.c_void_p), ('workspace_bytes', ctypes.c_int64),
    ]


class _ModconvPlanInfo(ctypes.Structure):
    _fields_ = [
        ('kind', ctypes.c_int32), ('tile_h', ctypes.c_int32), ('tile_w', ctypes.c_int32), ('images_per_tile', ctypes.c_int32),
        ('rows', ctypes.c_int32), ('waves', ctypes.c_int32), ('parts', ctypes.c_int32), ('f16', ctypes.c_int32),
        ('split_k', ctypes.c_int32), ('strip', ctypes.c_int32), ('transposed_all_class', ctypes.c_int32), ('reserved', ctypes.c_int32),
        ('workgroups', ctypes.c_int64),
    ]


PLAN_KINDS = ('fp32', 'split', 'split_teams', 'head_split', 'head_resident', 'head_small')

STYLE_BATCH_MAX = 24


class _StyleJob(ctypes.Structure):
    _fields_ = [
        ('w', ctypes.c_void_p), ('w_stride', ctypes.c_int64),
        ('affine_w', ctypes.c_void_p), ('affine_b', ctypes.c_void_p),
        ('wsq_t', ctypes.c_void_p),
        ('cin', ctypes.c_int32), ('cout', ctypes.c_int32),
        ('affine_gain', ctypes.c_float), ('bias_gain', ctypes.c_float),
        ('styles', ctypes.c_void_p), ('dcoefs', ctypes.c_void_p),
    ]


class _FoldJob(ctypes.Structure):
    _fields_ = [
        ('w', ctypes.c_void_p), ('w_stride', ctypes.c_int64),
        ('cin', ctypes.c_int32), ('affine_gain', ctypes.c_float),
        ('a0', ctypes.c_void_p), ('b0', ctypes.c_void_p), ('w0', ctypes.c_void_p), ('cout0', ctypes.c_int32), ('gain0', ctypes.c_float),
        ('a1', ctypes.c_void_p), ('b1', ctypes.c_void_p), ('w1', ctypes.c_void_p), ('cout1', ctypes.c_int32), ('gain1', ctypes.c_float),
        ('out', ctypes.c_void_p),
    ]


LOWRES_MAX_LAYERS, LOWRES_MAX_HEADS = 8, 4


class _LowresLayer(ctypes.Structure):
    _fields_ = [('weight', ctypes.c_void_p), ('styles', ctypes.c_void_p), ('dcoefs', ctypes.c_void_p), ('noise', ctypes.c_void_p), ('bias', ctypes.c_void_p),
                ('act_gain', ctypes.c_float), ('clamp', ctypes.c_float), ('up', ctypes.c_int32), ('head', ctypes.c_int32),
                ('weights_packed', ctypes.c_int32), ('reserved', ctypes.c_int32)]


class _LowresHead(ctypes.Structure):
    _fields_ = [('w', ctypes.c_void_p), ('bias', ctypes.c_void_p), ('skip', ctypes.c_void_p), ('clamp', ctypes.c_float), ('O', ctypes.c_int32)]


class _LowresParams(ctypes.Structure):
    _fields_ = [('x0', ctypes.c_void_p), ('x0_batch_stride', ctypes.c_int64), ('fir', ctypes.c_void_p), ('x_out', ctypes.c_void_p),
                ('workspace', ctypes.c_void_p), ('workspace_bytes', ctypes.c_int64),
                ('n', ctypes.c_int32), ('C', ctypes.c_int32), ('res0', ctypes.c_int32), ('nlayers', ctypes.c_int32), ('nheads', ctypes.c_int32),
                ('arith', ctypes.c_int32), ('reserved0', ctypes.c_int32), ('reserved', ctypes.c_int32),
                ('layers', _LowresLayer * LOWRES_MAX_LAYERS), ('heads', _LowresHead * LOWRES_MAX_HEADS)]


class _MappingParams(ctypes.Structure):
    _fields_ = [
        ('z', ctypes.c_void_p), ('c', ctypes.c_void_p), ('embed_w', ctypes.c_void_p), ('embed_b', ctypes.c_void_p),
        ('fc_w', ctypes.c_void_p * 16), ('fc_b', ctypes.c_void_p * 16), ('fc_out', ctypes.c_int32 * 16),
        ('w_avg', ctypes.c_void_p), ('ws', ctypes.c_void_p),
        ('workspace', ctypes.c_void_p), ('workspace_bytes', ctypes.c_int64),
        ('n', ctypes.c_int32), ('z_dim', ctypes.c_int32), ('c_dim', ctypes.c_int32), ('embed', ctypes.c_int32),
        ('layers', ctypes.c_int32), ('num_ws', ctypes.c_int32),
        ('embed_weight_gain', ctypes.c_float), ('embed_bias_gain', ctypes.c_float), ('lr_multiplier', ctypes.c_float),
        ('alpha', ctypes.c_float), ('act_gain', ctypes.c_float), ('truncation_psi', ctypes.c_float),
        ('truncation_cutoff', ctypes.c_int32),
    ]


LPIPS_MAX_TAPS = 8


class _LpipsTap(ctypes.Structure):
    _fields_ = [
        ('a', ctypes.c_void_p), ('t', ctypes.c_void_p), ('lin', ctypes.c_void_p), ('out', ctypes.c_void_p),
        ('c', ctypes.c_int32), ('h', ctypes.c_int32), ('w', ctypes.c_int32), ('reserved', ctypes.c_int32),
    ]


PARSE_JOIN_TERMS = 3
# ... 71 lines not shown
            'ide3d_triplane_sample_rays': [vp, ctypes.POINTER(i64 * 4), i32, i32, i32, i32, vp, i64, vp, i32, i32, i32, vp],
            'ide3d_triplane_taps': [i32, i32, vp, i64, vp, vp],
            'ide3d_triplane_sample_backward': [vp, vp, ctypes.POINTER(i64 * 4), i32, i32, i32, i32, vp, i64,
                                               vp, ctypes.POINTER(i64 * 4), vp, vp],
            'ide3d_composite': [vp, vp, vp, vp, i64, i32, i32, ctypes.c_int, ctypes.c_int, ctypes.c_int, f32,
                                ctypes.c_int, vp, vp, vp, vp],
            'ide3d_sample_pdf': [vp, vp, vp, i64, i64, i32, i32, f32, vp, vp],
            'ide3d_render_rays': [ctypes.POINTER(_RenderParams), vp],
            'ide3d_render_rays_backward': [ctypes.POINTER(_RenderParams), ctypes.POINTER(_RenderGrads), vp],
            'ide3d_render_param_grad_workspace_bytes': [ctypes.POINTER(_RenderParams)],
            'ide3d_render_rays_backward_params': [ctypes.POINTER(_RenderParams), ctypes.POINTER(_RenderGrads), ctypes.POINTER(_RenderParamGrads), vp],
            'ide3d_render_camera_grad_workspace_bytes': [ctypes.POINTER(_RenderParams)],
            'ide3d_render_rays_backward_camera': [ctypes.POINTER(_RenderParams), ctypes.POINTER(_RenderGrads), ctypes.POINTER(_RenderParamGrads),
                                                  ctypes.POINTER(_RenderCameraGrads), vp],
            'ide3d_sample_voxel': [ctypes.POINTER(_RenderParams), vp, i64, vp, vp, ctypes.c_int, vp],
            'ide3d_lattice_points': [ctypes.POINTER(_Lattice), i64, i64, vp, vp],
            'ide3d_density_lattice': [ctypes.POINTER(_RenderParams), ctypes.POINTER(_Lattice), i64, i64, vp, vp],
            'ide3d_modconv2d': [ctypes.POINTER(_ModconvParams), vp],
            'ide3d_modconv2d_heads': [ctypes.POINTER(_ModconvParams), ctypes.POINTER(_ModconvHeadEpilogue), vp],
            'ide3d_modconv_plan': [ctypes.POINTER(_ModconvParams), ctypes.POINTER(_ModconvPlanInfo)],
            'ide3d_modconv_workspace_bytes': [i32, i32, i32, i32, i32, i32, i32, i32],
            'ide3d_act_bwd_workspace_bytes': [i32, i32, i32, i32],
            'ide3d_modconv_act_backward': [ctypes.POINTER(_ActBwdParams), vp],
            'ide3d_modconv_scale_dot': [vp, vp, vp, vp, vp, i32, i32, i32, i32, vp, i64, vp],
            'ide3d_head_wgrad_workspace_bytes': [i32, i32, i32, i32, i32],
            'ide3d_head_weight_grad': [vp, vp, vp, i32, i32, i32, i32, i32, vp, i64, vp],
            'ide3d_wgrad_workspace_bytes': [i32, i32, i32, i32, i32],
            'ide3d_modconv_weight_grad': [ctypes.POINTER(_WgradParams), vp],
            'ide3d_bias_noise_workspace_bytes': [i32, i32, i32, i32],
            'ide3d_bias_noise_grad': [vp, vp, vp, i32, i32, i32, i32, vp, i64, vp],
            'ide3d_noise_reg_workspace_bytes': [ctypes.POINTER(i32), i32],
            'ide3d_noise_reg_levels': [ctypes.POINTER(i32), i32],
            'ide3d_noise_reg': [vp, ctypes.POINTER(i32), i32, vp, i64, vp, vp, vp],
            'ide3d_noise_reg_backward': [vp, ctypes.POINTER(i32), i32, vp, i64, vp, vp, vp, vp],
            'ide3d_noise_normalize_workspace_bytes': [ctypes.POINTER(i32), i32],
            'ide3d_noise_normalize': [vp, ctypes.POINTER(i32), i32, vp, i64, vp],
            'ide3d_lpips_prep': [vp, vp, vp, vp, i32, i32, i32, i32, f32, f32, vp],
            'ide3d_lpips_prep_backward': [vp, vp, vp, i32, i32, i32, i32, f32, vp],
            'ide3d_maxpool2': [vp, vp, i64, i32, i32, vp],
            'ide3d_lpips_stage_backward': [vp, vp, vp, vp, i64, i32, i32, vp],
            'ide3d_lpips_head_workspace_bytes': [ctypes.POINTER(_LpipsTap), i32, i32],
            'ide3d_lpips_head': [ctypes.POINTER(_LpipsTap), i32, i32, vp, i64, vp, vp],
            'ide3d_lpips_head_backward': [ctypes.POINTER(_LpipsTap), i32, i32, vp, vp],
            'ide3d_unfold2d': [vp, vp, i32, i32, i32, i32, i32, i32, i32, vp],
            'ide3d_fold2d': [vp, vp, i32, i32, i32, i32, i32, i32, i32, vp],
            'ide3d_maxpool3s2p0': [vp, vp, vp, i64, i32, i32, vp],
            'ide3d_lpips_tap_backward': [vp, vp, vp, vp, vp, i64, i32, i32, i32, vp],
            'ide3d_resize_bilinear': [vp, vp, i64, i32, i32, i32, i32, vp],
            'ide3d_resize_bilinear_backward': [vp, vp, i64, i32, i32, i32, i32, vp],
            'ide3d_parse_ce_workspace_bytes': [i32, i32, i32, i32, i32, i32],
            'ide3d_parse_ce': [vp, vp, i32, i32, i32, i32, i32, i32, vp, vp, i64, vp, vp],
            'ide3d_parse_ce_backward': [vp, vp, vp, vp, vp, i32, i32, i32, i32, i32, i32, vp],
            'ide3d_maxpool3s2': [vp, vp, vp, i64, i32, i32, vp],
            'ide3d_maxpool3s2_backward': [vp, vp, vp, vp, i64, i32, i32, vp],
            'ide3d_parse_join': [ctypes.POINTER(_ParseJoinParams), vp],
            'ide3d_plane_sums': [vp, vp, vp, i64, i64, f32, vp],
            'ide3d_parse_stem_backward': [vp, vp, vp, i32, i32, i32, i32, vp],
            'ide3d_id_prep': [vp, vp, i32, i32, vp],
            'ide3d_id_prep_backward': [vp, vp, i32, i32, vp],
            'ide3d_prelu': [vp, vp, vp, i32, i32, i32, i32, vp],
            'ide3d_prelu_backward': [vp, i64, i64, i32, vp, vp, vp, i32, i32, i32, i32, vp],
            'ide3d_se_gate': [vp, vp, vp, vp, i32, i32, i32, vp],
            'ide3d_se_gate_backward': [vp, vp, vp, vp, vp, vp, i32, i32, i32, vp],
            'ide3d_linear_workspace_bytes': [i32, i32, i32],
            'ide3d_linear_backward_input_workspace_bytes': [i32, i32, i32],
            'ide3d_linear': [vp, vp, vp, vp, i32, i32, i32, vp, i64, vp],
            'ide3d_linear_backward_input': [vp, vp, vp, i32, i32, i32, vp, i64, vp],
            'ide3d_linear_weight_grad': [vp, vp, vp, i32, i32, i32, vp],
            'ide3d_residual_join': [vp, vp, vp, i64, f32, vp],
            'ide3d_id_head': [vp, vp, vp, vp, vp, i32, i32, vp],
            'ide3d_id_head_backward': [vp, vp, vp, vp, vp, i32, i32, vp],
            'ide3d_set_conv_arithmetic': [i32],
            'ide3d_get_conv_arithmetic': [],
            'ide3d_frame_u8': [vp, vp, vp, i32, i32, i32, i32, vp, vp],
            'ide3d_sphere_points': [vp, vp, i32, ctypes.c_float, i32, vp, vp, vp],
            'ide3d_cam2world': [vp, vp, vp, i32, i32, vp, vp],
            'ide3d_style_demod': [vp, i64, vp, vp, vp, i32, i32, i32, i32, f32, f32, vp, vp, vp],
            'ide3d_fold_heads': [vp, i64, i32, i32, i32, f32, vp, vp, vp, i32, f32, vp, vp, vp, i32, f32, vp, vp],
            'ide3d_style_demod_batch': [ctypes.POINTER(_StyleJob), i32, i32, i32, vp],
            'ide3d_fold_heads_batch': [ctypes.POINTER(_FoldJob), i32, i32, i32, vp],
            'ide3d_mapping': [ctypes.POINTER(_MappingParams), vp],
            'ide3d_mapping_workspace_bytes': [],
            'ide3d_mapping_supported': [],
            'ide3d_skip_upsample_add_cl': [vp, ctypes.POINTER(i64 * 4), vp, ctypes.POINTER(i64 * 4), i32, i32, i32, i32, vp, vp],
            'ide3d_bilinear_up2_split': [vp, i32, i32, i32, i32, ctypes.POINTER(vp * 3), ctypes.POINTER(i32 * 3), ctypes.POINTER(i32 * 3), ctypes.POINTER(ctypes.c_int64 * 3), vp],
            'ide3d_lowres_layers_supported': [i32, i32, i32, ctypes.POINTER(i32), i32, i32],
            'ide3d_lowres_workspace_bytes': [ctypes.POINTER(_LowresParams)],
            'ide3d_lowres_group': [ctypes.POINTER(_LowresParams), vp],
        }
        for name, argtypes in protos.items():
            fn = getattr(lib, name)
            fn.restype = ctypes.c_int64 if name.endswith('_bytes') else ctypes.c_int
            fn.argtypes = argtypes
        _lib = lib
        return _lib


EXPORTED_SYMBOLS = (
    'ide3d_last_error', 'ide3d_abi_version', 'ide3d_build_arch', 'ide3d_build_flags', 'ide3d_exclusive_violations', 'ide3d_exclusive_violation_text', 'ide3d_bias_act', 'ide3d_upfirdn2d', 'ide3d_upfirdn2d_ex',
    'ide3d_filtered_lrelu', 'ide3d_filtered_lrelu_act', 'ide3d_triplane_sample', 'ide3d_triplane_sample_rays', 'ide3d_triplane_taps',
    'ide3d_triplane_sample_backward', 'ide3d_composite', 'ide3d_sample_pdf', 'ide3d_render_rays', 'ide3d_render_rays_backward', 'ide3d_sample_voxel',
    'ide3d_lattice_points', 'ide3d_density_lattice',
    'ide3d_modconv2d', 'ide3d_modconv2d_heads', 'ide3d_modconv_workspace_bytes', 'ide3d_modconv_plan', 'ide3d_set_conv_arithmetic', 'ide3d_get_conv_arithmetic', 'ide3d_frame_u8', 'ide3d_sphere_points', 'ide3d_cam2world', 'ide3d_style_demod', 'ide3d_fold_heads',
    'ide3d_style_demod_batch', 'ide3d_fold_heads_batch',
    'ide3d_skip_upsample_add_cl', 'ide3d_bilinear_up2_split', 'ide3d_mapping', 'ide3d_mapping_workspace_bytes', 'ide3d_mapping_supported',
    'ide3d_lowres_layers_supported', 'ide3d_lowres_phase_r_plan', 'ide3d_lowres_workspace_bytes', 'ide3d_lowres_group',
    'ide3d_act_bwd_workspace_bytes', 'ide3d_modconv_act_backward', 'ide3d_modconv_scale_dot', 'ide3d_head_wgrad_workspace_bytes',
    'ide3d_head_weight_grad', 'ide3d_wgrad_workspace_bytes', 'ide3d_modconv_weight_grad', 'ide3d_bias_noise_workspace_bytes',
    'ide3d_bias_noise_grad', 'ide3d_render_param_grad_workspace_bytes', 'ide3d_render_rays_backward_params',
    'ide3d_noise_reg_workspace_bytes', 'ide3d_noise_reg_levels', 'ide3d_noise_reg', 'ide3d_noise_reg_backward',
    'ide3d_noise_normalize_workspace_bytes', 'ide3d_noise_normalize',
    'ide3d_render_camera_grad_workspace_bytes', 'ide3d_render_rays_backward_camera',
    'ide3d_lpips_prep', 'ide3d_lpips_prep_backward', 'ide3d_maxpool2', 'ide3d_lpips_stage_backward', 'ide3d_lpips_head_workspace_bytes',
    'ide3d_lpips_head', 'ide3d_lpips_head_backward',
    'ide3d_unfold2d', 'ide3d_fold2d', 'ide3d_maxpool3s2p0', 'ide3d_lpips_tap_backward',
    'ide3d_resize_bilinear', 'ide3d_resize_bilinear_backward', 'ide3d_parse_ce_workspace_bytes', 'ide3d_parse_ce', 'ide3d_parse_ce_backward',
    'ide3d_maxpool3s2', 'ide3d_maxpool3s2_backward', 'ide3d_parse_join', 'ide3d_plane_sums', 'ide3d_parse_stem_backward',
    'ide3d_id_prep', 'ide3d_id_prep_backward', 'ide3d_prelu', 'ide3d_prelu_backward', 'ide3d_se_gate', 'ide3d_se_gate_backward',
    'ide3d_linear_workspace_bytes', 'ide3d_linear_backward_input_workspace_bytes', 'ide3d_linear', 'ide3d_linear_backward_input',
    'ide3d_linear_weight_grad', 'ide3d_residual_join', 'ide3d_id_head', 'ide3d_id_head_backward',
)


def exclusive_violations():
    lib = load()
    lib.ide3d_exclusive_violations.restype = ctypes.c_int
    lib.ide3d_exclusive_violation_text.restype = ctypes.c_char_p
    return int(lib.ide3d_exclusive_violations()), lib.ide3d_exclusive_violation_text().decode('utf-8', 'replace')


def _check(rc, what):
    if rc == 0:
        CALLS[what] = CALLS.get(what, 0) + 1
    if rc != 0:
        msg = load().ide3d_last_error().decode('utf-8', 'replace')
        raise RuntimeError(f'{what} failed (code {rc}): {msg}')


_raw_stream = getattr(torch._C, '_cuda_getCurrentRawStream', None)


def _stream_handle(device):
    if _raw_stream is not None:
        return _raw_stream(device.index if device.index is not None else torch.cuda.current_device())
    return torch.cuda.current_stream(device).cuda_stream


def _stream(t):
    return ctypes.c_void_p(_stream_handle(t.device))


_private_streams = {}


def _hip_runtime():
    paths = _hip_runtimes_mapped()
    if len(paths) != 1:
        raise RuntimeError(f'expected exactly one HIP runtime mapped in this process, found {sorted(paths)}')
    rt = ctypes.CDLL(next(iter(paths)))
    rt.hipStreamCreateWithFlags.argtypes = [ctypes.POINTER(ctypes.c_void_p), ctypes.c_uint]
    rt.hipStreamCreateWithFlags.restype = ctypes.c_int
    return rt


def private_stream(device, purpose):
    device = torch.device(device)
    idx = device.index if device.index is not None else torch.cuda.current_device()
    key = (idx, purpose)
    st = _private_streams.get(key)
    if st is None:
        with _lock:
            st = _private_streams.get(key)
            if st is None:
                torch.cuda.init()
                h = ctypes.c_void_p()
                with torch.cuda.device(idx):
                    rc = _hip_runtime().hipStreamCreateWithFlags(ctypes.byref(h), 1)
                if rc != 0 or not h.value:
                    raise RuntimeError(f'hipStreamCreateWithFlags failed ({rc})')
                st = _private_streams[key] = torch.cuda.ExternalStream(h.value, device=torch.device('cuda', idx))
    return st


capture_lock = threading.RLock()


# ... 600 lines not shown
        sig = torch.empty([p.n * int(count)], dtype=torch.float32, device=tex_planes.device)
        if count:
            with _dev_guard(tex_planes.device):
                rc = load().ide3d_density_lattice(ctypes.byref(p), ctypes.byref(lat), int(first), int(count), _ptr(sig), _stream(tex_planes))
            if rc == -2:
                return None
            _check(rc, 'density_lattice')
        return sig


class ModconvPlugin:
    _ws = _Workspaces(limit=1024)
    _heads_declined = set()

    @staticmethod
    def _workspace(lib, x, w, n, cin, cout, h, wd, k, mode, per_image, arith):
        key = (0 if per_image else w.data_ptr(), tuple(w.shape), n, h, wd, mode, x.device.index, _ws_domain(x.device), arith)
        def alloc():
            nbytes = lib.ide3d_modconv_workspace_bytes(n, cin, cout, h, wd, k, mode, int(per_image))
            _require(nbytes >= 0, 'modconv2d: unsupported configuration')
            return torch.empty([max(nbytes // 4, 1)], dtype=torch.float32, device=x.device)
        return ModconvPlugin._ws.entry(key, alloc)

    @staticmethod
    def _params(lib, x, w, y, styles, dcoefs, noise, noise_strength, bias, act, alpha, gain, clamp, mode, arith, x_amax, y_amax):
        n, cin, h, wd = x.shape
        per_image = (w.ndim == 5)
        cout, _, k, _ = w.shape[-4:]
        ent = ModconvPlugin._workspace(lib, x, w, n, cin, cout, h, wd, k, mode, per_image, arith)
        p = _ModconvParams()
        p.x, p.w, p.y = x.data_ptr(), w.data_ptr(), (y.data_ptr() if y is not None else None)
        keep = []
        for name, t in (('styles', styles), ('dcoefs', dcoefs), ('noise', noise), ('bias', bias)):
            if t is not None:
                t = t.contiguous(); keep.append(t)
                _require(t.is_cuda and t.dtype == torch.float32, f'modconv2d: {name} must be float32 on GPU')
                _require(t.device == x.device, f'modconv2d: {name} must reside on the same device as x')
                setattr(p, name, t.data_ptr())
        p.n, p.cin, p.cout, p.h, p.w_, p.k = n, cin, cout, h, wd, k
        p.noise_strength = float(noise_strength)
        p.act, p.alpha, p.gain, p.clamp = int(act), float(alpha), float(gain), float(clamp)
        p.mode = mode
        p.weights_packed = int((not per_image) and ModconvPlugin._ws.packed(ent, (w,))[0])
        p.w_batch_stride = (cout * cin * k * k) if per_image else 0
        p.arith = arith
        for name, t in (('x_amax', x_amax), ('y_amax', y_amax)):
            if t is not None:
                _require(t.is_cuda and t.device == x.device and t.dtype == torch.float32 and tuple(t.shape) == (n, AMAX_FLOATS) and t.is_contiguous(),
                         f'modconv2d: {name} must be a contiguous float32 [n, AMAX_FLOATS] tensor on the device of x')
                setattr(p, name, t.data_ptr())
        p.workspace, p.workspace_bytes = ent[0].data_ptr(), ent[0].numel() * 4
        return p, ent, keep

    @staticmethod
    def modconv2d(x, w, styles, dcoefs, noise, noise_strength, bias, act, alpha, gain, clamp, mode=0, arith=0, x_amax=None, y_amax=None, pad_rows=False):
        for t in (x, w):
            _require(t.is_cuda and t.dtype == torch.float32 and t.is_contiguous(), 'modconv2d: contiguous float32 CUDA tensors required')
        _require(w.device == x.device, 'modconv2d: w must reside on the same device as x')
        n, cin, h, wd = x.shape
        per_image = (w.ndim == 5)
        if per_image:
            _require(w.shape[0] == n and styles is None, 'modconv2d: per-image weights need w.shape[0] == batch and styles=None')
        cout, cin2, k, k2 = w.shape[-4:]
        _require(cin == cin2 and k == k2 and k in (1, 3), 'modconv2d: weight must be [cout, cin, k, k] with k in {1, 3}')
        _require(mode in (0, 1, 2), 'modconv2d: mode must be 0, 1 or 2')
        _require(mode != 1 or (k == 3 and h >= 3 and wd >= 3), 'modconv2d: mode 1 is a 3x3 stride-2 convolution on an input of at least 3x3')
        oh, ow = (2 * h + 1, 2 * wd + 1) if mode == 2 else (((h - 3) // 2 + 1, (wd - 3) // 2 + 1) if mode == 1 else (h, wd))
        pitch = (ow + 3) // 4 * 4 if (pad_rows and mode == 2) else ow
        y = torch.empty([n, cout, oh, pitch], dtype=torch.float32, device=x.device)
        lib = load()
        arith = int(arith) or int(lib.ide3d_get_conv_arithmetic())
        if arith == 16 and x_amax is None:
            arith = 6
        p, ent, keep = ModconvPlugin._params(lib, x, w, y, styles, dcoefs, noise, noise_strength, bias, act, alpha, gain, clamp, mode, arith, x_amax, y_amax)
        p.y_pitch = pitch if pitch != ow else 0
        with _dev_guard(x.device):
            rc = lib.ide3d_modconv2d(ctypes.byref(p), _stream(x))
        _check(rc, 'modconv2d')
        ModconvPlugin._ws.mark_packed(ent, () if per_image else (w,))
        return y if pitch == ow else y[..., :ow]

    @staticmethod
    def modconv2d_heads(x, w, styles, dcoefs, noise, noise_strength, bias, act, alpha, gain, clamp, head_w, head_bias, head_clamp,
                        want_x=True, arith=0):
        for t in (x, w, head_w):
            _require(t.is_cuda and t.dtype == torch.float32 and t.is_contiguous(), 'modconv2d_heads: contiguous float32 CUDA tensors required')
        n, cin, h, wd = x.shape
        cout = w.shape[0]
        _require(w.ndim == 4 and tuple(w.shape[1:]) == (cin, 3, 3), 'modconv2d_heads: w must be [cout, cin, 3, 3]')
        _require(head_w.ndim == 5 and head_w.shape[0] == n and head_w.shape[2] == cout and tuple(head_w.shape[3:]) == (1, 1),
                 'modconv2d_heads: head_w must be [n, rows, cout, 1, 1]')
        lib = load()
        arith = int(arith) or int(lib.ide3d_get_conv_arithmetic())
        if arith == 16:
            arith = 6
        rows = head_w.shape[1]
        shape_key = (n, cin, cout, h, wd, rows, arith)
        knob_off = 'IDE3D_MODCONV_NO_HEAD_FUSION' in os.environ
        if knob_off or shape_key in ModconvPlugin._heads_declined:
            return None
        y = torch.empty([n, cout, h, wd], dtype=torch.float32, device=x.device) if want_x else None
        heads = torch.empty([n, rows, h, wd], dtype=torch.float32, device=x.device)
        p, ent, keep = ModconvPlugin._params(lib, x, w, y, styles, dcoefs, noise, noise_strength, bias, act, alpha, gain, clamp, 0, arith, None, None)
        hent = ModconvPlugin._workspace(lib, heads, head_w, n, cout, rows, h, wd, 1, 0, True, arith)
        e = _ModconvHeadEpilogue()
        e.w, e.y, e.rows, e.clamp, e.no_activation_output = head_w.data_ptr(), heads.data_ptr(), rows, float(head_clamp), int(not want_x)
        if head_bias is not None:
            head_bias = head_bias.contiguous()
            _require(head_bias.is_cuda and head_bias.dtype == torch.float32 and head_bias.numel() == rows, 'modconv2d_heads: head_bias must be float32 [rows] on GPU')
            e.bias = head_bias.data_ptr()
        e.workspace, e.workspace_bytes = hent[0].data_ptr(), hent[0].numel() * 4
        with _dev_guard(x.device):
            rc = lib.ide3d_modconv2d_heads(ctypes.byref(p), ctypes.byref(e), _stream(x))
        if rc == -2:
            ModconvPlugin._heads_declined.add(shape_key)
            return None
        _check(rc, 'modconv2d_heads')
        ModconvPlugin._ws.mark_packed(ent, (w,))
        return y, heads


class ModconvGradPlugin:

    @staticmethod
    def _f32(t, name, dev, shape=None):
        _require(t.is_cuda and t.dtype == torch.float32 and t.device == dev, f'{name} must be float32 on the device of the gradient')
        if shape is not None:
            _require(tuple(t.shape) == tuple(shape), f'{name} must be {list(shape)}, got {list(t.shape)}')
        return t

    @staticmethod
    def act_backward(dy, y, act, alpha, gain, clamp, noise=None, noise_strength=1.0, bias=None, dcoefs=None):
        dev = dy.device
        ModconvGradPlugin._f32(dy, 'dy', dev)
        _require(dy.ndim == 4 and dy.is_contiguous(), 'act_backward: dy must be a contiguous [n, c, h, w] tensor')
        n, c, h, w = dy.shape
        ModconvGradPlugin._f32(y, 'y', dev, dy.shape)
        _require(y.stride(3) == 1 and y.stride(2) >= w and y.stride(1) == h * y.stride(2) and y.stride(0) == c * y.stride(1),
                 'act_backward: y must be dense apart from padded rows')
        _require(act in (0, 1, 3), 'act_backward: act must be 0 (dot only), 1 (linear) or 3 (lrelu)')
        _require(act != 0 or dcoefs is not None, 'act_backward: the dot-only form needs dcoefs')
        lib = load()
        p = _ActBwdParams()
        keep = []
        p.dy, p.y = dy.data_ptr(), y.data_ptr()
        p.y_pitch = y.stride(2) if y.stride(2) != w else 0
        dz = torch.empty_like(dy) if act != 0 else None
        if dz is not None:
            p.dz = dz.data_ptr()
        if noise is not None:
            noise = ModconvGradPlugin._f32(noise, 'noise', dev).contiguous(); keep.append(noise)
            _require(noise.numel() == h * w, 'act_backward: noise must be [h, w]')
            p.noise = noise.data_ptr()
        p.noise_strength = float(noise_strength)
        if bias is not None:
            bias = ModconvGradPlugin._f32(bias, 'bias', dev, (c,)).contiguous(); keep.append(bias)
            p.bias = bias.data_ptr()
        dd = ws = None
        if dcoefs is not None:
            dcoefs = ModconvGradPlugin._f32(dcoefs, 'dcoefs', dev, (n, c)).contiguous(); keep.append(dcoefs)
            dd = torch.empty([n, c], dtype=torch.float32, device=dev)
            nbytes = lib.ide3d_act_bwd_workspace_bytes(n, c, h, w)
            _require(nbytes > 0, 'act_backward: unsupported shape')
            ws = torch.empty([nbytes // 4], dtype=torch.float32, device=dev)
            p.dcoefs, p.ddcoefs, p.workspace, p.workspace_bytes = dcoefs.data_ptr(), dd.data_ptr(), ws.data_ptr(), nbytes
        p.n, p.c, p.h, p.w = n, c, h, w
        p.act, p.alpha, p.gain, p.clamp = int(act), float(alpha), float(gain), float(clamp)
        with _dev_guard(dev):
            rc = lib.ide3d_modconv_act_backward(ctypes.byref(p), _stream(dy))
        _check(rc, 'modconv_act_backward')
        return dz, dd

    @staticmethod
    def scale_dot(x, t, styles):
        dev = t.device
        ModconvGradPlugin._f32(t, 't', dev)
        _require(t.ndim == 4 and t.is_contiguous(), 'scale_dot: t must be a contiguous [n, c, h, w] tensor')
        n, c, h, w = t.shape
        x = ModconvGradPlugin._f32(x, 'x', dev, t.shape).contiguous()
        styles = ModconvGradPlugin._f32(styles, 'styles', dev, (n, c)).contiguous()
        lib = load()
        dx = torch.empty_like(t)
        ds = torch.empty([n, c], dtype=torch.float32, device=dev)
        nbytes = lib.ide3d_act_bwd_workspace_bytes(n, c, h, w)
        _require(nbytes > 0, 'scale_dot: unsupported shape')
        ws = torch.empty([nbytes // 4], dtype=torch.float32, device=dev)
        with _dev_guard(dev):
            rc = lib.ide3d_modconv_scale_dot(_ptr(x), _ptr(t), _ptr(styles), _ptr(dx), _ptr(ds), n, c, h, w, _ptr(ws), nbytes, _stream(t))
        _check(rc, 'modconv_scale_dot')
        return dx, ds

    @staticmethod
    def head_weight_grad(dy, x):
        dev = dy.device
        ModconvGradPlugin._f32(dy, 'dy', dev)
        _require(dy.ndim == 4 and x.ndim == 4 and x.shape[0] == dy.shape[0] and x.shape[2:] == dy.shape[2:], 'head_weight_grad: dy [n, rows, h, w], x [n, cin, h, w]')
        dy = dy.contiguous()
        x = ModconvGradPlugin._f32(x, 'x', dev).contiguous()
        n, rows, h, w = dy.shape
        cin = x.shape[1]
# ... 1097 lines not shown
```

### ide-3d_amd/training/networks.py

```python

import math

import numpy as np
import torch

from dnnlib import util
from torch_utils import custom_ops
from torch_utils import misc
from torch_utils import persistence
from torch_utils.ops import bias_act
from torch_utils.ops import conv2d_resample
from torch_utils.ops import fma
from torch_utils.ops import upfirdn2d

_modconv_plugin = None

use_hip_modconv = True


def _upfirdn_plugin():
    upfirdn2d._init()
    return upfirdn2d._plugin


# ... 440 lines not shown
    if not (lay.weight.shape[2:] == (3, 3) and lay.padding == 1 and lay.up in (1, 2) and lay.activation in ('linear', 'lrelu') and x.ndim == 4
            and styles.shape[0] == x.shape[0]):
        return None
    oh, ow = lay.up * x.shape[2], lay.up * x.shape[3]
    noise_const = getattr(lay, 'noise_const', None)
    map_grad = noise_const is not None and noise_const.requires_grad
    map_used = map_grad and noise is not None and noise.ndim == 2 and tuple(noise_const.shape) == (oh, ow)
    if (map_grad and not (hip_noise_grad and map_used)) or not _conv_grad_ok(x, styles, *_layer_params(lay), noise_map=(noise_const if map_used else None)):
        return None
    gh, gw = (oh + 1, ow + 1) if lay.up == 2 else (oh, ow)
    if x.shape[0] * lay.weight.shape[0] * gh * gw >= 2 ** 31 or x.numel() >= 2 ** 31:
        return None
    if noise is not None and not (noise.ndim == 2 and tuple(noise.shape) == (oh, ow) and (hip_param_grad or map_used or not noise.requires_grad)):
        return None
    if lay.resample_filter.requires_grad:
        return None
    if dcoefs is None:
        dcoefs = _demod_coefs(lay.weight, styles)
    bias = lay.bias.to(x.dtype)
    if lay.up == 1:
        return _ModconvActGrad.apply(x, styles, dcoefs, lay.weight, noise, bias, lay.activation, act_gain, act_clamp)
    return _ModconvUpGrad.apply(x, styles, dcoefs, lay.weight, lay.resample_filter, noise, bias, lay.activation, act_gain, act_clamp)


def _folded_head_weights(torgb, toseg, w):
    if not (w.ndim == 2 and w.stride(1) == 1 and torgb.weight.shape[2] == 1
            and _inference_on_gpu(w, torgb.weight, toseg.weight, torgb.affine.weight, torgb.affine.bias, toseg.affine.weight, toseg.affine.bias)
            and _style_init()):
        return None
    return _style_plugin.fold_heads(w, torgb.affine.weight_gain,
                                    torgb.affine.weight, torgb.affine.bias, torgb.weight.reshape(torgb.weight.shape[0], -1), torgb.weight_gain,
                                    toseg.affine.weight, toseg.affine.bias, toseg.weight.reshape(toseg.weight.shape[0], -1), toseg.weight_gain)


def _adjacent_views(a, b):
    if a is None or b is None or a._base is None or a._base is not b._base:
        return None
    t = a._base
    if (t.ndim != 4 or a.ndim != 4 or b.ndim != 4 or not t.is_contiguous() or t.shape[1] != a.shape[1] + b.shape[1]
            or a.shape[0] != t.shape[0] or a.shape[2:] != t.shape[2:] or b.shape[0] != t.shape[0] or b.shape[2:] != t.shape[2:]
            or a.stride() != t.stride() or b.stride() != t.stride()
            or a.data_ptr() != t.data_ptr() or b.data_ptr() != t.data_ptr() + a.shape[1] * t.stride(1) * t.element_size()):
        return None
    return t


def _dual_head_weights(torgb, toseg, w):
    wcat = _take_prefetched(torgb, w) if _prefetch_table() else None
    if wcat is None:
        wcat = _folded_head_weights(torgb, toseg, w)
    if wcat is None:
        s_rgb = torgb.affine(w) * torgb.weight_gain
        s_seg = toseg.affine(w) * toseg.weight_gain
        wr = torgb.weight[None, :, :, 0, 0] * s_rgb[:, None, :]
        ws = toseg.weight[None, :, :, 0, 0] * s_seg[:, None, :]
        wcat = torch.cat([wr, ws], dim=1)[:, :, :, None, None].contiguous()
    return wcat


def _dual_head(x, torgb, toseg, w, wcat=None):
    if (hip_conv_grad and torch.is_grad_enabled() and torgb.weight.shape[2] == 1 and torgb.conv_clamp == toseg.conv_clamp and x.ndim == 4
            and w.ndim == 2 and w.shape[0] == x.shape[0] and x.numel() < 2 ** 31
            and x.shape[0] * (torgb.weight.shape[0] + toseg.weight.shape[0]) * x.shape[2] * x.shape[3] < 2 ** 31
            and _conv_grad_ok(x, w, *_head_params(torgb, toseg))):
        y = _DualHeadGrad.apply(x, _dual_head_weights(torgb, toseg, w), _cat_cached(torgb.bias, toseg.bias),
                                -1.0 if torgb.conv_clamp is None else torgb.conv_clamp)
        co = torgb.weight.shape[0]
        return y[:, :co], y[:, co:]
    if not (use_hip_modconv and torgb.weight.shape[2] == 1 and torgb.conv_clamp == toseg.conv_clamp
            and _inference_on_gpu(x, w, *_head_params(torgb, toseg)) and _modconv_init()):
        return None
    n = x.shape[0]
    if w.shape[0] != n:
        return None
    if wcat is None:
        wcat = _dual_head_weights(torgb, toseg, w)
    bias = _cat_cached(torgb.bias, toseg.bias)
    clamp = -1.0 if torgb.conv_clamp is None else torgb.conv_clamp
    y = _modconv_plugin.modconv2d(x.contiguous(), wcat, None, None, None, 0.0, bias, 1, 0.0, 1.0, clamp)
    co = torgb.weight.shape[0]
    return y[:, :co], y[:, co:]


def _conv1_dual_head(block, x, w1, w_shared, want_x, noise_mode='random', gain=1, input_noise=None, **unused):
    c1, tr, ts = block.conv1, block.torgb, block.toseg
    if not (use_hip_modconv and type(c1) is SynthesisLayer and c1.up == 1 and c1.padding == 1 and c1.weight.shape[2:] == (3, 3)
            and c1.activation in ('linear', 'lrelu') and tr.weight.shape[2] == 1 and tr.conv_clamp == ts.conv_clamp
            and x.ndim == 4 and x.shape[0] == w1.shape[0] == w_shared.shape[0]
            and _inference_on_gpu(x, w1, w_shared, *_layer_params(c1), *_head_params(tr, ts))
            and not _hooked(block, c1, tr, ts) and _modconv_init()):
        return None
    from torch_utils import hip_plugin
    if hip_plugin.conv_arithmetic() != 'bf16x6':
        return None
    noise = None
    if c1.use_noise and noise_mode != 'none':
        if input_noise is not None or noise_mode != 'const' or tuple(c1.noise_const.shape) != tuple(x.shape[2:]):
            return None
        noise = _scaled_const_noise(c1.noise_const, c1.noise_strength)
    styles, dcoefs = _styles_and_dcoefs(c1.affine, w1, c1.weight, True)
    if dcoefs is None:
        dcoefs = _demod_coefs(c1.weight, styles)
    spec = bias_act.activation_funcs[c1.activation]
    act_gain = c1.act_gain * gain
    act_clamp = c1.conv_clamp * gain if c1.conv_clamp is not None else None
    bias = c1.bias.to(x.dtype)
    wcat = _dual_head_weights(tr, ts, w_shared)
    hbias = _cat_cached(tr.bias, ts.bias)
    hclamp = -1.0 if tr.conv_clamp is None else tr.conv_clamp
    xc = x.contiguous()
    out = _modconv_plugin.modconv2d_heads(xc, c1.weight.contiguous(), styles.contiguous(), dcoefs, noise, 1.0, bias,
                                          spec.cuda_idx, spec.def_alpha, act_gain, -1.0 if act_clamp is None else act_clamp,
                                          wcat, hbias, hclamp, want_x=want_x)
    if out is None:
        x = _modconv_bias_act(x, c1.weight, styles, True, noise, 1.0, bias, c1.activation, act_gain, act_clamp, dcoefs=dcoefs)
        return x, _dual_head(x, tr, ts, w_shared, wcat=wcat)
    x, y = out
    co = tr.weight.shape[0]
    return x, (y[:, :co], y[:, co:])


_lowres_plugin = None


def _lowres_init():
    global _lowres_plugin
    if _lowres_plugin is None:
        _lowres_plugin = custom_ops.get_plugin(module_name='lowres_plugin', sources=['lowres.hip'])
    return True


def _hooked(*modules):
    from torch.nn.modules import module as _m
    if _m._global_forward_hooks or _m._global_forward_pre_hooks:
        return True
    return any(m._forward_hooks or m._forward_pre_hooks for m in modules)


def lowres_group_forward(blocks, ws_per_block, noise_mode='const', force_fp32=False, **other_kwargs):
    if os.environ.get('IDE3D_NO_LOWRES_GROUP') or not use_hip_modconv or other_kwargs or noise_mode not in ('const', 'none'):
        return None
    if not blocks or len(blocks) != len(ws_per_block):
        return None
    b0 = blocks[0]
    ws0 = ws_per_block[0]
    if not (torch.is_tensor(ws0) and ws0.is_cuda and ws0.dtype == torch.float32) or (torch.is_grad_enabled() and ws0.requires_grad):
        return None
    if b0.in_channels != 0 or b0.use_single_layer or not hasattr(b0, 'const') or not _inference_on_gpu(b0.const, b0.conv1.weight):
        return None
    from torch_utils import hip_plugin
    if hip_plugin.conv_arithmetic() not in ('bf16x6', 'bf16x3'):
        return None
    C, n = b0.out_channels, ws0.shape[0]
    if C % 32 != 0 or n > 8:
        return None
    cand = []
    for bi, blk in enumerate(blocks):
        ok = (blk.architecture == 'skip' and not blk.use_single_layer and blk.out_channels == C and (bi == 0 or blk.in_channels == C)
              and not (blk.use_fp16 and not force_fp32) and not getattr(blk, 'skip_channels_last', False)
              and blk.torgb.conv_clamp == blk.toseg.conv_clamp and blk.torgb.weight.shape[2] == 1 and blk._filter_is_1331()
              and blk.resolution == b0.resolution << bi
              and not _hooked(blk, blk.conv1, blk.torgb, blk.toseg, *([blk.conv0] if bi else [])))
        if ok and torch.is_grad_enabled():
            ok = _inference_on_gpu(ws_per_block[bi], *([blk.const] if bi == 0 else _layer_params(blk.conv0)), *_layer_params(blk.conv1),
                                   *_head_params(blk.torgb, blk.toseg))
        if not ok:
            break
        for name in (('conv1',) if bi == 0 else ('conv0', 'conv1')):
            lay = getattr(blk, name)
            if not (lay.activation == 'lrelu' and lay.weight.shape == (C, C, 3, 3) and lay.padding == 1 and lay.up == (2 if name == 'conv0' else 1)
                    and _inference_on_gpu(ws0, lay.weight, lay.bias) and lay.weight.is_contiguous()
                    and (not lay.use_noise or noise_mode == 'none' or lay.noise_const.shape[-1] == blk.resolution)):
                ok = False
                break
            cand.append((bi, name, lay))
        if not ok:
            cand = [c for c in cand if c[0] < bi]
            break
    if not cand or not _lowres_init():
        return None
    ups = [lay.up for _, _, lay in cand]
    fit = _lowres_plugin.layers_supported(n, C, b0.resolution, ups)
    if fit < 1:
        return None
    cand = cand[:fit]
    last_bi, last_name, _ = cand[-1]
    resume = last_name == 'conv0'
    nheads = last_bi if resume else last_bi + 1
    if nheads > hip_plugin.LOWRES_MAX_HEADS or (nheads == 0):
        return None
    layers, heads = [], []
    for bi, name, lay in cand:
        blk, wsb = blocks[bi], ws_per_block[bi]
        w = wsb[:, (0 if (bi == 0 or name == 'conv0') else 1)]
        styles, dcoefs = _styles_and_dcoefs(lay.affine, w, lay.weight, True)
        noise = None
        if lay.use_noise and noise_mode == 'const':
            noise = _scaled_const_noise(lay.noise_const, lay.noise_strength)
        layers.append(dict(weight=lay.weight, styles=styles, dcoefs=dcoefs, noise=noise, bias=lay.bias, act_gain=lay.act_gain,
                           clamp=(-1.0 if lay.conv_clamp is None else lay.conv_clamp), up=lay.up,
                           head=(bi if (name == 'conv1' and bi < nheads) else -1)))
    for bi in range(nheads):
        blk, wsb = blocks[bi], ws_per_block[bi]
# ... 385 lines not shown
        return bias_act.bias_act(x, self.bias.to(x.dtype), act=self.activation, gain=act_gain, clamp=act_clamp)


@persistence.persistent_class
class ToRGBLayer(torch.nn.Module):

    def __init__(self, in_channels, out_channels, w_dim, kernel_size=1, conv_clamp=None, channels_last=False, **unused):
        super().__init__()
        self.conv_clamp = conv_clamp
        self.affine = FullyConnectedLayer(w_dim, in_channels, bias_init=1)
        memory_format = torch.channels_last if channels_last else torch.contiguous_format
        self.weight = torch.nn.Parameter(torch.randn([out_channels, in_channels, kernel_size, kernel_size]).to(memory_format=memory_format))
        self.bias = torch.nn.Parameter(torch.zeros([out_channels]))
        self.weight_gain = 1 / np.sqrt(in_channels * (kernel_size ** 2))

    def forward(self, x, w, fused_modconv=True):
        styles = self.affine(w) * self.weight_gain
        if x.size(0) > styles.size(0):
            assert x.size(0) % styles.size(0) == 0
            styles = styles.repeat_interleave(x.size(0) // styles.size(0), dim=0)
        y = _modconv_bias_act(x, self.weight, styles, False, None, 0.0, self.bias.to(x.dtype), 'linear', 1.0, self.conv_clamp)
        if y is not None:
            return y
        x = modulated_conv2d(x=x, weight=self.weight, styles=styles, demodulate=False, fused_modconv=fused_modconv)
        return bias_act.bias_act(x, self.bias.to(x.dtype), clamp=self.conv_clamp)


@persistence.persistent_class
class SegSynthesisBlock(torch.nn.Module):

    def __init__(self, in_channels, out_channels, w_dim, resolution, img_channels, seg_channels, is_last,
                 architecture='skip', resample_filter=[1, 3, 3, 1], conv_clamp=None, use_fp16=False,
                 fp16_channels_last=False, use_single_layer=False, disable_upsample=False, **layer_kwargs):
        assert architecture in ['orig', 'skip']
        super().__init__()
        self.in_channels, self.out_channels = in_channels, out_channels
        self.w_dim, self.resolution = w_dim, resolution
        self.img_channels, self.seg_channels = img_channels, seg_channels
        self.is_last, self.architecture = is_last, architecture
        self.use_fp16 = use_fp16
        self.channels_last = (use_fp16 and fp16_channels_last)
        self.use_single_layer = use_single_layer
        self.register_buffer('resample_filter', upfirdn2d.setup_filter(resample_filter))
        self.num_conv = self.num_torgb = self.num_toseg = 0
        layer_name = layer_kwargs.pop('layer_name', 'training.networks.SynthesisLayer')

        if in_channels == 0:
            self.const = torch.nn.Parameter(torch.randn([out_channels, resolution, resolution]))
        else:
            self.conv0 = util.construct_class_by_name(
                class_name=layer_name, in_channels=in_channels, out_channels=out_channels, w_dim=w_dim,
                resolution=resolution, up=(1 if disable_upsample else 2), resample_filter=resample_filter,
                conv_clamp=conv_clamp, channels_last=self.channels_last, **layer_kwargs)
            self.num_conv += 1
        if not use_single_layer:
            self.conv1 = util.construct_class_by_name(
                class_name=layer_name, in_channels=out_channels, out_channels=out_channels, w_dim=w_dim,
                resolution=resolution, conv_clamp=conv_clamp, channels_last=self.channels_last, **layer_kwargs)
            self.num_conv += 1
        if is_last or architecture == 'skip':
            self.torgb = ToRGBLayer(out_channels, img_channels, w_dim=w_dim, conv_clamp=conv_clamp, channels_last=self.channels_last)
            self.num_torgb += 1
            self.toseg = ToRGBLayer(out_channels, seg_channels, w_dim=w_dim, conv_clamp=conv_clamp, channels_last=self.channels_last)
            self.num_toseg += 1

    def _merge_skip(self, skip, x):
        if skip is None:
            return None
        if skip.size(-1) * 2 == x.size(-1):
            return upfirdn2d.upsample2d(skip, self.resample_filter)
        if skip.size(-1) == x.size(-1):
            return skip
        raise NotImplementedError

    def _accumulate(self, lo, cur, y):
        if lo is not None:
            if (getattr(self, 'skip_channels_last', False) and lo.shape[1] % 4 == 0 and self.resample_filter.shape == (4, 4)
                    and _inference_on_gpu(lo, y) and self._filter_is_1331() and _resample_init()):
                return _resample_plugin.skip_upsample_add_cl(lo, y)
            f = self.resample_filter
            return _upfirdn_plugin().upfirdn2d_ex(lo, f, 2, 2, 1, 1, 2, 1, 2, 1, False, 4.0, add=y)
        return cur.add_(y) if cur is not None else y

    def _filter_is_1331(self):
        ok = getattr(self, '_f1331', None)
        if ok is None:
            ref = upfirdn2d.setup_filter([1, 3, 3, 1])
            ok = self._f1331 = bool(torch.equal(self.resample_filter.detach().cpu(), ref))
        return ok

    def forward(self, x, img, seg, ws, force_fp32=False, fused_modconv=None, block_noise=None, disable_rgb=False, **layer_kwargs):
        misc.assert_shape(ws, [None, self.num_conv + self.num_torgb, self.w_dim])
        resume_after_conv0 = bool(layer_kwargs.pop('_resume_after_conv0', False))
        x_unused = bool(layer_kwargs.pop('_x_unused', False))
        ws_list = ws.unbind(dim=1)
        w_iter = iter(ws_list)
        dtype = torch.float16 if self.use_fp16 and not force_fp32 else torch.float32
        memory_format = torch.channels_last if self.channels_last and not force_fp32 else torch.contiguous_format
        out_dtype = dtype
        if dtype == torch.float16 and ws.is_cuda and not torch.is_grad_enabled() and use_hip_modconv:
            dtype, memory_format = torch.float32, torch.contiguous_format
        if fused_modconv is None:
            with misc.suppress_tracer_warnings():
                fused_modconv = (not self.training) and (dtype == torch.float32 or int(ws.shape[0]) == 1)

        fused = fused_heads = None
        if self.in_channels == 0:
            x = self.const.to(dtype=dtype, memory_format=memory_format)
            x = x.unsqueeze(0).expand(ws.shape[0], *x.size())
            if not self.use_single_layer:
                layer_kwargs['input_noise'] = block_noise[:, 1:2] if block_noise is not None else None
                x = self.conv1(x, next(w_iter), fused_modconv=fused_modconv, **layer_kwargs)
        else:
            x = x.to(dtype=dtype, memory_format=memory_format)
            layer_kwargs['input_noise'] = block_noise[:, 0:1] if block_noise is not None else None
            if resume_after_conv0:
                next(w_iter)
            else:
                x = self.conv0(x, next(w_iter), fused_modconv=fused_modconv, **layer_kwargs)
            if not self.use_single_layer:
                layer_kwargs['input_noise'] = block_noise[:, 1:2] if block_noise is not None else None
                w1 = next(w_iter)
                if (self.is_last or self.architecture == 'skip') and not disable_rgb and dtype == torch.float32:
                    fused = _conv1_dual_head(self, x, w1, ws_list[self.num_conv], not x_unused, **layer_kwargs)
                if fused is not None:
                    x, fused_heads = fused
                else:
                    x = self.conv1(x, w1, fused_modconv=fused_modconv, **layer_kwargs)

        w_shared = next(w_iter) if (self.is_last or self.architecture == 'skip') else None
        ref = x if x is not None else fused_heads[0]
        img_lo = seg_lo = None
        heads_follow = (self.is_last or self.architecture == 'skip') and not disable_rgb
        if (heads_follow and _inference_on_gpu(ref, img, seg, w_shared, *_head_params(self.torgb, self.toseg)) and img is not None and seg is not None
                and img.size(-1) * 2 == ref.size(-1)):
            img_lo, seg_lo, img, seg = img, seg, None, None
        else:
            img = self._merge_skip(img, ref)
            seg = self._merge_skip(seg, ref)
        if self.is_last or self.architecture == 'skip':
            if disable_rgb:
                img = seg = None
            else:
                heads = fused_heads if fused_heads is not None else _dual_head(x, self.torgb, self.toseg, w_shared)
                if heads is not None:
                    y, y_seg = heads
                else:
                    y = self.torgb(x, w_shared, fused_modconv=fused_modconv).to(dtype=torch.float32, memory_format=torch.contiguous_format)
                    y_seg = self.toseg(x, w_shared, fused_modconv=fused_modconv).to(dtype=torch.float32, memory_format=torch.contiguous_format)
                lo_both, y_both = _adjacent_views(img_lo, seg_lo), _adjacent_views(y, y_seg)
                if (lo_both is not None and y_both is not None and img is None and seg is None and not getattr(self, 'skip_channels_last', False)
                        and not self.is_last and not os.environ.get('IDE3D_NO_SKIP_MERGE')):
                    both = self._accumulate(lo_both, None, y_both)
                    img, seg = both[:, :y.shape[1]], both[:, y.shape[1]:]
                else:
                    img = self._accumulate(img_lo, img, y)
                    seg = self._accumulate(seg_lo, seg, y_seg)
        assert x is None or x.dtype == dtype
        if x is not None and out_dtype != dtype:
            x = x.to(out_dtype)
        assert img is None or img.dtype == torch.float32
        assert seg is None or seg.dtype == torch.float32
        return x, img, seg
```

### include/ide3d_hip.h

```cpp
#ifndef IDE3D_HIP_H_
#define IDE3D_HIP_H_

#include <stdint.h>

#ifdef __cplusplus
extern "C" {
#endif


#define IDE3D_OK            0
#define IDE3D_EINVAL       (-1)
#define IDE3D_ENOKERNEL    (-2)
#define IDE3D_ELAUNCH      (-3)

#define IDE3D_F32  0
#define IDE3D_F16  1
#define IDE3D_BF16 2
#define IDE3D_F64  3

const char* ide3d_last_error(void);
int         ide3d_abi_version(void);
const char* ide3d_build_arch(void);
const char* ide3d_build_flags(void);
int         ide3d_exclusive_violations(void);
// ... 123 lines not shown
    float   max_depth;
    float*  out_feat;
    float*  out_depth;
    float*  out_wsum;
} ide3d_render_params;

int ide3d_render_rays(const ide3d_render_params* p, void* stream);

typedef struct ide3d_render_grads {
    const float* grad_feat;  const float* grad_depth;  const float* grad_wsum;
    float* grad_tex_planes;  float* grad_geo_planes;
    int64_t grad_tex_stride[4];  int64_t grad_geo_stride[4];
} ide3d_render_grads;

int ide3d_render_rays_backward(const ide3d_render_params* p, const ide3d_render_grads* g, void* stream);

typedef struct ide3d_render_param_grads {
    float* grad_geo_w0; float* grad_geo_b0; float* grad_geo_w1; float* grad_geo_b1;
    float* grad_tex_w0; float* grad_tex_b0; float* grad_tex_w1; float* grad_tex_b1;
    void* workspace;
    int64_t workspace_bytes;
} ide3d_render_param_grads;

int64_t ide3d_render_param_grad_workspace_bytes(const ide3d_render_params* p);
int ide3d_render_rays_backward_params(const ide3d_render_params* p, const ide3d_render_grads* g, const ide3d_render_param_grads* q, void* stream);

typedef struct ide3d_render_camera_grads {
    float* grad_cam2world;
    void* workspace;
    int64_t workspace_bytes;
} ide3d_render_camera_grads;

int64_t ide3d_render_camera_grad_workspace_bytes(const ide3d_render_params* p);
int ide3d_render_rays_backward_camera(const ide3d_render_params* p, const ide3d_render_grads* g, const ide3d_render_param_grads* q,
                                      const ide3d_render_camera_grads* c, void* stream);

int ide3d_sample_voxel(const ide3d_render_params* p, const float* pts, int64_t m,
                       float* out, float* out_sigma, int sigma_only, void* stream);

typedef struct ide3d_lattice {
    int32_t n;
    float   voxel_size;
    float   corner[3];
    float   scale;
} ide3d_lattice;

int ide3d_lattice_points(const ide3d_lattice* lat, int64_t first, int64_t count, float* pts, void* stream);

int ide3d_density_lattice(const ide3d_render_params* p, const ide3d_lattice* lat, int64_t first, int64_t count,
                          float* out_sigma, void* stream);

typedef struct ide3d_modconv_params {
    const float* x; const float* w; const float* styles; const float* dcoefs;
    const float* noise; const float* bias; float* y;
    int32_t n, cin, cout, h, w_, k;
    float noise_strength;
    int32_t act; float alpha, gain, clamp;
    int32_t mode;
    int32_t weights_packed;
    float*  workspace;
    int64_t workspace_bytes;
    int64_t w_batch_stride;
    int32_t arith;
    const float* x_amax;
    float*       y_amax;
    int32_t      y_pitch;
} ide3d_modconv_params;

int64_t ide3d_modconv_workspace_bytes(int32_t n, int32_t cin, int32_t cout, int32_t h, int32_t w, int32_t k, int32_t mode,
                                      int32_t per_image_weights);
int ide3d_modconv2d(const ide3d_modconv_params* p, void* stream);

typedef struct ide3d_modconv_head_epilogue {
    const float* w;
    const float* bias;
    float*       y;
    int32_t      rows;
    float        clamp;
    int32_t      no_activation_output;
    float*       workspace;
    int64_t      workspace_bytes;
} ide3d_modconv_head_epilogue;
int ide3d_modconv2d_heads(const ide3d_modconv_params* p, const ide3d_modconv_head_epilogue* heads, void* stream);

typedef struct ide3d_act_bwd_params {
    const float* dy;
    const float* y;
    float*       dz;
    const float* noise;
    float        noise_strength;
    const float* bias;
    const float* dcoefs;
    float*       ddcoefs;
    int32_t      n, c, h, w, y_pitch;
    int32_t      act;
    float        alpha, gain, clamp;
    float*       workspace;
    int64_t      workspace_bytes;
} ide3d_act_bwd_params;

int64_t ide3d_act_bwd_workspace_bytes(int32_t n, int32_t c, int32_t h, int32_t w);
int ide3d_modconv_act_backward(const ide3d_act_bwd_params* p, void* stream);

int ide3d_modconv_scale_dot(const float* x, const float* t, const float* styles, float* dx, float* dstyles,
                            int32_t n, int32_t c, int32_t h, int32_t w, float* workspace, int64_t workspace_bytes, void* stream);

int64_t ide3d_head_wgrad_workspace_bytes(int32_t n, int32_t rows, int32_t cin, int32_t h, int32_t w);
int ide3d_head_weight_grad(const float* dy, const float* x, float* dw, int32_t n, int32_t rows, int32_t cin, int32_t h, int32_t w,
                           float* workspace, int64_t workspace_bytes, void* stream);

typedef struct ide3d_wgrad_params {
    const float* g;
    const float* x;
    const float* styles;
    const float* dcoefs;
    float*       dw;
    int32_t      n, cin, cout, h, w;
    int32_t      mode;
    int32_t      arith;
    float*       workspace;
    int64_t      workspace_bytes;
} ide3d_wgrad_params;

int64_t ide3d_wgrad_workspace_bytes(int32_t n, int32_t cin, int32_t cout, int32_t h, int32_t w);
int ide3d_modconv_weight_grad(const ide3d_wgrad_params* p, void* stream);

int64_t ide3d_bias_noise_workspace_bytes(int32_t n, int32_t c, int32_t h, int32_t w);
int ide3d_bias_noise_grad(const float* dz, float* db, float* dnoise, int32_t n, int32_t c, int32_t h, int32_t w,
                          float* workspace, int64_t workspace_bytes, void* stream);

enum { IDE3D_PLAN_FP32 = 0,
       IDE3D_PLAN_SPLIT = 1,
       IDE3D_PLAN_SPLIT_TEAMS = 2,
       IDE3D_PLAN_HEAD_SPLIT = 3,
       IDE3D_PLAN_HEAD_RESIDENT = 4,
       IDE3D_PLAN_HEAD_SMALL = 5 };
typedef struct ide3d_modconv_plan_info {
    int32_t kind;
    int32_t tile_h, tile_w;
    int32_t images_per_tile;
    int32_t rows;
    int32_t waves;
    int32_t parts, f16;
    int32_t split_k;
    int32_t strip;
    int32_t transposed_all_class;
    int32_t reserved;
    int64_t workgroups;
} ide3d_modconv_plan_info;
int ide3d_modconv_plan(const ide3d_modconv_params* p, ide3d_modconv_plan_info* out);

int     ide3d_set_conv_arithmetic(int32_t arith);
int32_t ide3d_get_conv_arithmetic(void);

int ide3d_style_demod(const float* w, int64_t w_stride, const float* affine_w, const float* affine_b, const float* wsq_t,
                      int32_t n, int32_t cin, int32_t cout, int32_t wdim, float affine_gain, float bias_gain,
                      float* styles, float* dcoefs, void* stream);

int ide3d_fold_heads(const float* w, int64_t w_stride, int32_t n, int32_t cin, int32_t wdim, float affine_gain,
                     const float* a0, const float* b0, const float* w0, int32_t cout0, float gain0,
                     const float* a1, const float* b1, const float* w1, int32_t cout1, float gain1,
                     float* out, void* stream);

#define IDE3D_STYLE_BATCH_MAX 24
typedef struct ide3d_style_job {
    const float* w; int64_t w_stride;
// ... 190 lines not shown
```

Before: 957.9 frames/s.

## Fuse skip-branch upsample-and-add into the fused conv1+heads kernel epilogue

Adds a skip epilogue to the split-bf16 conv1+toRGB/toSeg head kernel. The kernel loads a low-resolution RGB/seg window, applies the 2x [1,3,3,1] upsample taps and adds the head outputs before writing the final skip images. This removes the separate upfirdn/merge kernels and the intermediate head-output round trip through memory. In exchange it adds a new kernel variant with extra LDS staging and two syncs. The channels-last form stays disabled by default.

```diff
diff --git a/ide-3d_amd/csrc/modconv.hip b/ide-3d_amd/csrc/modconv.hip
--- a/ide-3d_amd/csrc/modconv.hip
+++ b/ide-3d_amd/csrc/modconv.hip
@@ -1,5 +1,6 @@
 #include "common.h"
 #include "knobs.h"
+#include "skip_blend.h"
 #include <stdlib.h>
 #include <string.h>
 #include <type_traits>
@@ -602,9 +603,16 @@
     int store_x;
     int bias_first;
 };
-template <int PH, int PW, int NWV, int MTW, int NTW, int BM, int MT, int PARTS, int SCRATCH>
+struct SkipEpi {
+    const float* lo[2];
+    int64_t lo_s[2][4];
+    float* out[2];
+    int64_t out_bs[2];
+    int c[2];
+};
+template <int PH, int PW, int NWV, int MTW, int NTW, int BM, int MT, int PARTS, int SCRATCH, int SKIP = 0>
 __device__ __forceinline__ void split_heads_finish(const ide3d_modconv_params& p, const HeadEpi& he, f32x16 (&acc)[1][MTW][NTW], float* smem,
-                                                   int n0, int y0, int x0, int wm, int wn, int lp) {
+                                                   int n0, int y0, int x0, int wm, int wn, int lp, const SkipEpi* sk = nullptr) {
     constexpr int NT = 64 * NWV, BN = PH * PW, TP = BN + 4, ROWS = MT * 32, CCH = BM / 16, A_UNITS = PARTS * 2 * ROWS;
     static_assert(BM * TP + 2 * BM + ROWS <= SCRATCH, "activation tile + coefficients must fit the loop's LDS");
     const int tid = threadIdx.x, lane = tid & 63, half = lane >> 5, l32 = lane & 31;
@@ -670,6 +678,26 @@
 #pragma unroll
                 for (int k = 0; k < 4; ++k) hacc[m][t][4 * g + k] = he.bias_first ? b4[k] : 0.f;
         }
+    constexpr int LO_H = PH / 2 + 2, LO_W = PW / 2 + 2, LO_WIN = LO_H * LO_W, LO_N = SKIP ? (ROWS * LO_WIN + NT - 1) / NT : 1;
+    static_assert(!SKIP || ROWS * LO_WIN <= BM * TP, "the skip window takes the place of the activation tile");
+    float lo_v[LO_N];
+    auto fetch_lo = [&]() {
+        const int lh = p.h >> 1, lw = p.w_ >> 1, m0 = (y0 >> 1) - 1, q0 = (x0 >> 1) - 1;
+        int t0 = tid;
+        asm volatile("" : "+v"(t0));
+#pragma unroll
+        for (int i = 0; i < LO_N; ++i) {
+            const int e = t0 + i * NT;
+            const int row = e / LO_WIN, r = e % LO_WIN, yy = m0 + r / LO_W, xx = q0 + r % LO_W;
+            const bool ok = row < he.rows && yy >= 0 && yy < lh && xx >= 0 && xx < lw;
+            const int rr = min(row, he.rows - 1), k = rr >= sk->c[0] ? 1 : 0, ch = rr - (k ? sk->c[0] : 0);
+            const float* src = k ? sk->lo[1] : sk->lo[0];
+            const int64_t* st = sk->lo_s[k];
+            const float v = src[n0 * st[0] + ch * st[1] + min(max(yy, 0), lh - 1) * st[2] + min(max(xx, 0), lw - 1) * st[3]];
+            lo_v[i] = ok ? v : 0.f;
+        }
+    };
+    if constexpr (SKIP && MT == 1) fetch_lo();
     u32x4 af[2][MTH][PARTS];
     auto fetch_a = [&](int c, int buf) {
 #pragma unroll
@@ -703,6 +731,69 @@
         }
     }
     const float h_clamp = (he.clamp >= 0.f) ? he.clamp : __builtin_inff();
+    auto head_finish = [&](float v, int row) {
+        if (he.bias_first) {
+            v = __builtin_amdgcn_fmed3f(v, -h_clamp, h_clamp);
+        } else {
+            v *= 1.f; v += 0.f; v += s_hb[row];
+            v = (v > 0.f) ? v : v * 1.f;
+            v = fminf(fmaxf(v, -h_clamp), h_clamp);
+        }
+        return v;
+    };
+    if constexpr (SKIP) {
+        if constexpr (MT != 1) fetch_lo();
+        __syncthreads();
+        float* const s_lo = s_t;
+#pragma unroll
+        for (int i = 0; i < LO_N; ++i) {
+            const int e = tid + i * NT;
+            if (e < ROWS * LO_WIN) s_lo[e] = lo_v[i];
+        }
+        __syncthreads();
+#pragma unroll
+        for (int t = 0; t < NTH; ++t) {
+            const int pix = (pg * NTH + t) * 32 + l32;
+            const int py = pix / PW, px = pix % PW, gy = y0 + py, gx = x0 + px;
+            const float* const wsrc = s_lo + ((py >> 1) + (py & 1)) * LO_W + (px >> 1) + (px & 1);
+            const float wy0 = (gy & 1) ? 0.75f : 0.25f, wy1 = 1.0f - wy0;
+            const float wx0 = (gx & 1) ? 0.75f : 0.25f, wx1 = 1.0f - wx0;
+            const float ga = wy0 * wx0, gb = wy0 * wx1, gc = wy1 * wx0, gd = wy1 * wx1;
+#pragma unroll
+            for (int m = 0; m < MTH; ++m)
+#pragma unroll
+                for (int g4 = 0; g4 < 4; ++g4) {
+                    const int row0 = (rg * MTH + m) * 32 + 8 * g4 + 4 * half;
+                    if (row0 >= he.rows) continue;
+                    float u[4];
+#pragma unroll
+                    for (int j = 0; j < 4; ++j) {
+                        const int row = row0 + j;
+                        const float* w = wsrc + row * LO_WIN;
+                        const float a = w[0], b = w[1], c = w[LO_W], d = w[LO_W + 1];
+                        float v;
+                        if constexpr (SKIP == 2) v = skip_cl_blend(wy0, wy1, wx0, wx1, a, b, c, d);
+                        else v = fir_up2_taps(a, b, c, d, ga, gb, gc, gd);
+                        v += head_finish(hacc[m][t][4 * g4 + j], row);
+                        u[j] = v;
+                    }
+                    if constexpr (SKIP == 2) {
+                        const int k = row0 >= sk->c[0] ? 1 : 0, ck = k ? sk->c[1] : sk->c[0];
+                        const f32x4a v4 = {u[0], u[1], u[2], u[3]};
+                        __builtin_nontemporal_store(v4, reinterpret_cast<f32x4a*>((k ? sk->out[1] : sk->out[0]) + (((int64_t)n0 * p.h + gy) * p.w_ + gx) * ck
+                                                                                  + row0 - (k ? sk->c[0] : 0)));
+                    } else {
+#pragma unroll
+                        for (int j = 0; j < 4; ++j) {
+                            const int row = row0 + j, kj = row >= sk->c[0] ? 1 : 0;
+                            if (row >= he.rows) continue;
+                            float* const o = (kj ? sk->out[1] : sk->out[0]) + n0 * (kj ? sk->out_bs[1] : sk->out_bs[0]);
+                            o[(int64_t)(row - (kj ? sk->c[0] : 0)) * hw + gy * p.w_ + gx] = u[j];
+                        }
+                    }
+                }
+        }
+    } else {
 #pragma unroll
     for (int t = 0; t < NTH; ++t) {
         const int pix = (pg * NTH + t) * 32 + l32;
@@ -714,24 +805,18 @@
             for (int r = 0; r < 16; ++r) {
                 const int row = (rg * MTH + m) * 32 + 8 * (r >> 2) + 4 * half + (r & 3);
                 if (row >= he.rows) continue;
-                float v = hacc[m][t][r];
-                if (he.bias_first) {
-                    v = __builtin_amdgcn_fmed3f(v, -h_clamp, h_clamp);
-                } else {
-                    v *= 1.f; v += 0.f; v += s_hb[row];
-                    v = (v > 0.f) ? v : v * 1.f;
-                    v = fminf(fmaxf(v, -h_clamp), h_clamp);
-                }
-                o[(int64_t)row * hw] = v;
+                o[(int64_t)row * hw] = head_finish(hacc[m][t][r], row);
             }
     }
+    }
     __syncthreads();
 }
 
-template <int MODE, int BIG, int PH, int PARTS, int WBUF, int NWV, int F16, int TEAMS = 1, int PAR = -1, int HEAD_MT = 0>
+template <int MODE, int BIG, int PH, int PARTS, int WBUF, int NWV, int F16, int TEAMS = 1, int PAR = -1, int HEAD_MT = 0, int SKIP = 0>
 __device__ __forceinline__ void modconv_split_tile(const ide3d_modconv_params& p, const u32x4* __restrict__ wp, float* __restrict__ partial,
                                                    const ConvGeom& g, unsigned char* smem, int mb, int tl, int grp, int split, int tiles_x,
-                                                   const float* __restrict__ row_unscale, float* wg_scratch = nullptr, const HeadEpi* he = nullptr) {
+                                                   const float* __restrict__ row_unscale, float* wg_scratch = nullptr, const HeadEpi* he = nullptr,
+                                                   const SkipEpi* sk = nullptr) {
     using K = SpCfg<MODE, BIG, PH, PARTS, WBUF, NWV, (PAR >= 0)>;
     static_assert(!F16 || PARTS == 2, "f16x3 = two fp16 pieces per operand");
     static_assert(PAR < 0 || (MODE == MODE_TCONV3A && WBUF == 2 && TEAMS == 1), "row-parity pairs: transposed form, two weight buffers, one team");
@@ -942,7 +1027,7 @@
 #endif
     if constexpr (HEAD_MT > 0) {
         static_assert(MODE == MODE_CONV3 && TEAMS == 1 && !F16 && K::NCLS == 1, "fused heads: 3x3 split-bf16 layers");
-        split_heads_finish<PH, PW, K::NWV, K::MTW, K::NTW, K::BM, HEAD_MT, PARTS, K::LDS_BYTES / 4>(p, *he, acc, reinterpret_cast<float*>(smem), n0, y0, x0, wm, wn, lp);
+        split_heads_finish<PH, PW, K::NWV, K::MTW, K::NTW, K::BM, HEAD_MT, PARTS, K::LDS_BYTES / 4, SKIP>(p, *he, acc, reinterpret_cast<float*>(smem), n0, y0, x0, wm, wn, lp, sk);
     } else
     modconv_finish<MODE, 1, PH, PW, K::NWV, K::NCLS, K::MTW, K::NTW, K::BM, K::LDS_BYTES / 4, PAR>(p, partial, g, acc, reinterpret_cast<float*>(smem), mb, n0, y0, x0, split, 0, wm, wn, lp,
                                                                                                 F16 ? row_unscale : nullptr, xus, (TEAMS == 2) ? tid : -1, wg_scratch);
@@ -1430,6 +1515,16 @@
     __shared__ __attribute__((aligned(16))) unsigned char sp_smem[K::LDS_BYTES];
     const BlockId b = decode_block(g);
     modconv_split_tile<MODE_CONV3, BIG, PH, 3, 2, 8, 0, 1, -1, HEAD_MT>(p, wp, nullptr, g, sp_smem, b.mb, b.tile, b.grp, b.split, g.tiles_x[0], nullptr, nullptr, &he);
+}
+
+template <int BIG, int PH, int HEAD_MT, int SKIP>
+__global__ void __launch_bounds__(512, 2)
+modconv_split_heads_skip_kernel(ide3d_modconv_params p, const u32x4* __restrict__ wp, ConvGeom g, HeadEpi he, SkipEpi sk) {
+    using K = SpCfg<MODE_CONV3, BIG, PH, 3, 2, 8>;
+    if constexpr (kSpExclusive) asm volatile("" ::: "v255");
+    __shared__ __attribute__((aligned(16))) unsigned char sp_smem[K::LDS_BYTES];
+    const BlockId b = decode_block(g);
+    modconv_split_tile<MODE_CONV3, BIG, PH, 3, 2, 8, 0, 1, -1, HEAD_MT, SKIP>(p, wp, nullptr, g, sp_smem, b.mb, b.tile, b.grp, b.split, g.tiles_x[0], nullptr, nullptr, &he, &sk);
 }
 
 template <int BIG, int PH, int PARTS, int F16 = 0>
@@ -1957,18 +2052,28 @@
     return IDE3D_OK;
 }
 
-extern "C" int ide3d_modconv2d_heads(const ide3d_modconv_params* pp, const ide3d_modconv_head_epilogue* hp, void* stream) {
+static int modconv2d_heads_impl(const ide3d_modconv_params* pp, const ide3d_modconv_head_epilogue* hp, const ide3d_modconv_skip_epilogue* sp, void* stream) {
     using namespace ide3d;
     IDE3D_CHECK_ARG(pp != nullptr && hp != nullptr, "modconv2d_heads: null params");
     const ide3d_modconv_params& p = *pp;
     const ide3d_modconv_head_epilogue& h = *hp;
-    IDE3D_CHECK_ARG(p.x && p.w && p.workspace && (p.y || h.no_activation_output) && h.w && h.y && h.workspace, "modconv2d_heads: null tensor / workspace pointer");
+    IDE3D_CHECK_ARG(p.x && p.w && p.workspace && (p.y || h.no_activation_output) && h.w && (h.y || sp) && h.workspace, "modconv2d_heads: null tensor / workspace pointer");
     int rc = check_modconv(p);
     if (rc) return rc;
     IDE3D_CHECK_ARG(p.act == 1 || p.act == 3, "modconv2d_heads: act must be linear (1) or lrelu (3)");
     IDE3D_CHECK_ARG(h.rows > 0, "modconv2d_heads: bad head rows");
     auto no_kernel = [](const char* why) { set_error("modconv2d_heads: %s", why); return IDE3D_ENOKERNEL; };
     if (knob_live("IDE3D_MODCONV_NO_HEAD_FUSION")) return no_kernel("IDE3D_MODCONV_NO_HEAD_FUSION is set");
+    if (sp) {
+        const ide3d_modconv_skip_epilogue& s = *sp;
+        IDE3D_CHECK_ARG(s.channels[0] > 0 && s.channels[1] >= 0 && s.channels[0] + s.channels[1] == h.rows, "modconv2d_heads_skip: channels must add up to the head rows");
+        for (int k = 0; k < 2; ++k)
+            IDE3D_CHECK_ARG(s.channels[k] == 0 || (s.lo[k] && s.out[k]), "modconv2d_heads_skip: null skip image %d", k);
+        IDE3D_CHECK_ARG(!s.channels_last || (s.channels[0] % 4 == 0 && s.channels[1] % 4 == 0 && (reinterpret_cast<uintptr_t>(s.out[0]) & 15) == 0 &&
+                                            (reinterpret_cast<uintptr_t>(s.out[1]) & 15) == 0),
+                        "modconv2d_heads_skip: channels-last outputs need channel counts that are multiples of 4 and 16-byte alignment");
+        if (knob_live("IDE3D_MODCONV_NO_SKIP_FUSION")) return no_kernel("IDE3D_MODCONV_NO_SKIP_FUSION is set");
+    }
     if (p.k != 3 || p.mode != 0 || p.w_batch_stride != 0 || p.y_amax || p.y_pitch != 0) return no_kernel("not a shared-weight 3x3 layer without side outputs");
     int arith = resolve_arith(p.arith);
     if (arith == 16 && !p.x_amax) arith = 6;
@@ -1987,6 +2092,7 @@
     const int mt = h.rows <= 32 ? 1 : 6, hcc = p.cout / 16;
     if (head_small_applies(q) || !head_split_applies(q, resolve_arith(q.arith)) || resolve_arith(q.arith) == 3 || (mt == 6 && !tile16))
         return no_kernel("the heads do not take the split-bf16 path");
+    if (sp && (sp->channels_last != 0) != (mt == 6)) return no_kernel("no fused skip form for this head size and output layout");
     IDE3D_CHECK_ARG(p.workspace_bytes >= (pl.packed_floats + pl.aux_floats) * (int64_t)sizeof(float), "modconv2d_heads: workspace too small");
     IDE3D_CHECK_ARG(h.workspace_bytes >= head_packed_units(p.n, hcc, 3, mt) * 16, "modconv2d_heads: head workspace too small");
     hipStream_t st = (hipStream_t)stream;
@@ -2000,11 +2106,32 @@
     const ConvGeom& g = pl.g;
     const unsigned nblocks = (unsigned)((int64_t)g.mblocks * g.tile_base[4] * g.img_groups * g.split_k);
     const u32x4* wu = reinterpret_cast<const u32x4*>(p.workspace);
+    if (sp) {
+        SkipEpi k;
+        for (int i = 0; i < 2; ++i) {
+            k.lo[i] = sp->lo[i]; k.out[i] = sp->out[i]; k.c[i] = sp->channels[i];
+            k.out_bs[i] = sp->out_batch_stride[i] ? sp->out_batch_stride[i] : (int64_t)sp->channels[i] * p.h * p.w_;
+            for (int d = 0; d < 4; ++d) k.lo_s[i][d] = sp->lo_stride[i][d];
+        }
+        if (tile32) IDE3D_EXCL_LAUNCH((modconv_split_heads_skip_kernel<2, 32, 1, 1>), dim3(nblocks), 512, 0, st, p, wu, g, e, k);
+        else if (mt == 1) IDE3D_EXCL_LAUNCH((modconv_split_heads_skip_kernel<1, 16, 1, 1>), dim3(nblocks), 512, 0, st, p, wu, g, e, k);
+        else IDE3D_EXCL_LAUNCH((modconv_split_heads_skip_kernel<1, 16, 6, 2>), dim3(nblocks), 512, 0, st, p, wu, g, e, k);
+        IDE3D_CHECK_LAUNCH("modconv2d_heads_skip");
+        return IDE3D_OK;
+    }
     if (tile32) IDE3D_EXCL_LAUNCH((modconv_split_heads_kernel<2, 32, 1>), dim3(nblocks), 512, 0, st, p, wu, g, e);
     else if (mt == 1) IDE3D_EXCL_LAUNCH((modconv_split_heads_kernel<1, 16, 1>), dim3(nblocks), 512, 0, st, p, wu, g, e);
     else IDE3D_EXCL_LAUNCH((modconv_split_heads_kernel<1, 16, 6>), dim3(nblocks), 512, 0, st, p, wu, g, e);
     IDE3D_CHECK_LAUNCH("modconv2d_heads");
     return IDE3D_OK;
+}
+
+extern "C" int ide3d_modconv2d_heads(const ide3d_modconv_params* pp, const ide3d_modconv_head_epilogue* hp, void* stream) {
+    return modconv2d_heads_impl(pp, hp, nullptr, stream);
+}
+extern "C" int ide3d_modconv2d_heads_skip(const ide3d_modconv_params* pp, const ide3d_modconv_head_epilogue* hp, const ide3d_modconv_skip_epilogue* sp, void* stream) {
+    IDE3D_CHECK_ARG(sp != nullptr, "modconv2d_heads_skip: null skip epilogue");
+    return modconv2d_heads_impl(pp, hp, sp, stream);
 }
 
 extern "C" int ide3d_modconv_plan(const ide3d_modconv_params* pp, ide3d_modconv_plan_info* out) {
diff --git a/ide-3d_amd/csrc/resample.hip b/ide-3d_amd/csrc/resample.hip
--- a/ide-3d_amd/csrc/resample.hip
+++ b/ide-3d_amd/csrc/resample.hip
@@ -1,4 +1,5 @@
 #include "common.h"
+#include "skip_blend.h"
 
 namespace ide3d {
 namespace {
@@ -65,7 +66,7 @@
 #pragma unroll
         for (int c = 0; c < SK_CH; ++c) {
             const float a = s_lo[c][ly][lx], bq = s_lo[c][ly][lx + 1], cq = s_lo[c][ly + 1][lx], d = s_lo[c][ly + 1][lx + 1];
-            float v = wy0 * (wx0 * a + wx1 * bq) + wy1 * (wx0 * cq + wx1 * d);
+            float v = skip_cl_blend(wy0, wy1, wx0, wx1, a, bq, cq, d);
             if (ok && c0 + c < p.c) v += add_v[c];
             s_t[tid][c] = v;
         }
diff --git a/ide-3d_amd/csrc/skip_blend.h b/ide-3d_amd/csrc/skip_blend.h
--- /dev/null
+++ b/ide-3d_amd/csrc/skip_blend.h
@@ -0,0 +1,18 @@
+#pragma once
+
+namespace ide3d {
+
+__device__ __forceinline__ float skip_cl_blend(float wy0, float wy1, float wx0, float wx1, float a, float b, float c, float d) {
+    return wy0 * (wx0 * a + wx1 * b) + wy1 * (wx0 * c + wx1 * d);
+}
+
+__device__ __forceinline__ float fir_up2_taps(float a, float b, float c, float d, float ga, float gb, float gc, float gd) {
+    float acc = 0.f;
+    acc += a * ga;
+    acc += b * gb;
+    acc += c * gc;
+    acc += d * gd;
+    return acc;
+}
+
+}
diff --git a/ide-3d_amd/csrc/upfirdn2d.hip b/ide-3d_amd/csrc/upfirdn2d.hip
--- a/ide-3d_amd/csrc/upfirdn2d.hip
+++ b/ide-3d_amd/csrc/upfirdn2d.hip
@@ -1,5 +1,6 @@
 #include "common.h"
 #include "knobs.h"
+#include "skip_blend.h"
 #include <type_traits>
 
 namespace ide3d {
@@ -579,13 +580,9 @@
                 for (int cx = 0; cx < 2; ++cx)
 #pragma unroll
                     for (int rx = 0; rx < 2; ++rx) {
-                        float acc = 0.f;
-#pragma unroll
-                        for (int ty_ = 0; ty_ < 2; ++ty_)
-#pragma unroll
-                            for (int tx_ = 0; tx_ < 2; ++tx_)
-                                acc += win[cy + AX::off(ry) + ty_][cx + AX::off(rx) + tx_] * g[AX::first(ry) + ty_ * 2][AX::first(rx) + tx_ * 2];
-                        row[cx * 2 + rx] = acc;
+                        const int wy = cy + AX::off(ry), wx = cx + AX::off(rx), fy = AX::first(ry), fx = AX::first(rx);
+                        row[cx * 2 + rx] = fir_up2_taps(win[wy][wx], win[wy][wx + 1], win[wy + 1][wx], win[wy + 1][wx + 1],
+                                                        g[fy][fx], g[fy][fx + 2], g[fy + 2][fx], g[fy + 2][fx + 2]);
                     }
                 if (has_add) {
                     const float4 a = *reinterpret_cast<const float4*>(ap + ((unsigned)oy * apitch + (unsigned)ox0));
diff --git a/ide-3d_amd/torch_utils/hip_plugin.py b/ide-3d_amd/torch_utils/hip_plugin.py
--- a/ide-3d_amd/torch_utils/hip_plugin.py
+++ b/ide-3d_amd/torch_utils/hip_plugin.py
@@ -163,6 +163,20 @@
         ('rows', ctypes.c_int32), ('clamp', ctypes.c_float), ('no_activation_output', ctypes.c_int32),
         ('workspace', ctypes.c_void_p), ('workspace_bytes', ctypes.c_int64),
     ]
+
+
+class _ModconvSkipEpilogue(ctypes.Structure):
+    _fields_ = [
+        ('lo', ctypes.c_void_p * 2), ('lo_stride', (ctypes.c_int64 * 4) * 2), ('out', ctypes.c_void_p * 2),
+        ('out_batch_stride', ctypes.c_int64 * 2), ('channels', ctypes.c_int32 * 2), ('channels_last', ctypes.c_int32), ('reserved', ctypes.c_int32),
+    ]
+
+
+class SkipImages(tuple):
+
+    @property
+    def shape(self):
+        return (self[0].shape[0], sum(t.shape[1] for t in self), *self[0].shape[2:])
 
 
 class _ModconvPlanInfo(ctypes.Structure):
@@ -400,6 +414,7 @@
             'ide3d_mapping': [ctypes.POINTER(_MappingParams), vp],
             'ide3d_mapping_workspace_bytes': [],
             'ide3d_mapping_supported': [],
+            'ide3d_modconv2d_heads_skip': [ctypes.POINTER(_ModconvParams), ctypes.POINTER(_ModconvHeadEpilogue), ctypes.POINTER(_ModconvSkipEpilogue), vp],
             'ide3d_skip_upsample_add_cl': [vp, ctypes.POINTER(i64 * 4), vp, ctypes.POINTER(i64 * 4), i32, i32, i32, i32, vp, vp],
             'ide3d_bilinear_up2_split': [vp, i32, i32, i32, i32, ctypes.POINTER(vp * 3), ctypes.POINTER(i32 * 3), ctypes.POINTER(i32 * 3), ctypes.POINTER(ctypes.c_int64 * 3), vp],
             'ide3d_lowres_layers_supported': [i32, i32, i32, ctypes.POINTER(i32), i32, i32],
@@ -419,7 +434,7 @@
     'ide3d_filtered_lrelu', 'ide3d_filtered_lrelu_act', 'ide3d_triplane_sample', 'ide3d_triplane_sample_rays', 'ide3d_triplane_taps',
     'ide3d_triplane_sample_backward', 'ide3d_composite', 'ide3d_sample_pdf', 'ide3d_render_rays', 'ide3d_render_rays_backward', 'ide3d_sample_voxel',
     'ide3d_lattice_points', 'ide3d_density_lattice',
-    'ide3d_modconv2d', 'ide3d_modconv2d_heads', 'ide3d_modconv_workspace_bytes', 'ide3d_modconv_plan', 'ide3d_set_conv_arithmetic', 'ide3d_get_conv_arithmetic', 'ide3d_frame_u8', 'ide3d_sphere_points', 'ide3d_cam2world', 'ide3d_style_demod', 'ide3d_fold_heads',
+    'ide3d_modconv2d', 'ide3d_modconv2d_heads', 'ide3d_modconv2d_heads_skip', 'ide3d_modconv_workspace_bytes', 'ide3d_modconv_plan', 'ide3d_set_conv_arithmetic', 'ide3d_get_conv_arithmetic', 'ide3d_frame_u8', 'ide3d_sphere_points', 'ide3d_cam2world', 'ide3d_style_demod', 'ide3d_fold_heads',
     'ide3d_style_demod_batch', 'ide3d_fold_heads_batch',
     'ide3d_skip_upsample_add_cl', 'ide3d_bilinear_up2_split', 'ide3d_mapping', 'ide3d_mapping_workspace_bytes', 'ide3d_mapping_supported',
     'ide3d_lowres_layers_supported', 'ide3d_lowres_phase_r_plan', 'ide3d_lowres_workspace_bytes', 'ide3d_lowres_group',
@@ -1186,7 +1201,7 @@
 
     @staticmethod
     def modconv2d_heads(x, w, styles, dcoefs, noise, noise_strength, bias, act, alpha, gain, clamp, head_w, head_bias, head_clamp,
-                        want_x=True, arith=0):
+                        want_x=True, arith=0, skip=None):
         for t in (x, w, head_w):
             _require(t.is_cuda and t.dtype == torch.float32 and t.is_contiguous(), 'modconv2d_heads: contiguous float32 CUDA tensors required')
         n, cin, h, wd = x.shape
@@ -1203,23 +1218,63 @@
         knob_off = 'IDE3D_MODCONV_NO_HEAD_FUSION' in os.environ
         if knob_off or shape_key in ModconvPlugin._heads_declined:
             return None
+        if skip is not None:
+            lo_img, lo_seg, layout = skip
+            _require(layout in ('joint', 'separate', 'channels_last'), 'modconv2d_heads: unknown skip layout')
+            ci, cs = lo_img.shape[1], lo_seg.shape[1]
+            for t, c in ((lo_img, ci), (lo_seg, cs)):
+                _require(t.is_cuda and t.dtype == torch.float32 and t.device == x.device and tuple(t.shape) == (n, c, h // 2, wd // 2),
+                         'modconv2d_heads: the low-resolution skip images must be float32 [n, c, h / 2, w / 2] on the device of x')
+            _require(ci + cs == rows and h % 2 == 0 and wd % 2 == 0, 'modconv2d_heads: the skip images\' channels must add up to the head rows')
+            skip_key = shape_key + (layout == 'channels_last',)
+            if skip_key in ModconvPlugin._heads_declined:
+                return None
         y = torch.empty([n, cout, h, wd], dtype=torch.float32, device=x.device) if want_x else None
-        heads = torch.empty([n, rows, h, wd], dtype=torch.float32, device=x.device)
+        e = _ModconvHeadEpilogue()
+        if skip is None:
+            heads = torch.empty([n, rows, h, wd], dtype=torch.float32, device=x.device)
+            e.y = heads.data_ptr()
+            ws_like = heads
+        else:
+            k = _ModconvSkipEpilogue()
+            if layout == 'channels_last':
+                _require(ci % 4 == 0 and cs % 4 == 0, 'modconv2d_heads: channels_last skip images need channel counts that are multiples of 4')
+                outs = [torch.empty([n, c, h, wd], dtype=torch.float32, device=x.device, memory_format=torch.channels_last) for c in (ci, cs)]
+                k.channels_last = 1
+            elif layout == 'joint':
+                both = torch.empty([n, rows, h, wd], dtype=torch.float32, device=x.device)
+                outs = [both[:, :ci], both[:, ci:]]
+            else:
+                outs = [torch.empty([n, c, h, wd], dtype=torch.float32, device=x.device) for c in (ci, cs)]
+            for i, (lo, out) in enumerate(zip((lo_img, lo_seg), outs)):
+                k.lo[i], k.out[i], k.channels[i] = lo.data_ptr(), out.data_ptr(), lo.shape[1]
+                k.out_batch_stride[i] = 0 if layout == 'channels_last' else out.stride(0)
+                for d in range(4):
+                    k.lo_stride[i][d] = lo.stride(d)
+            heads = SkipImages(outs)
+            ws_like = outs[0]
         p, ent, keep = ModconvPlugin._params(lib, x, w, y, styles, dcoefs, noise, noise_strength, bias, act, alpha, gain, clamp, 0, arith, None, None)
-        hent = ModconvPlugin._workspace(lib, heads, head_w, n, cout, rows, h, wd, 1, 0, True, arith)
-        e = _ModconvHeadEpilogue()
-        e.w, e.y, e.rows, e.clamp, e.no_activation_output = head_w.data_ptr(), heads.data_ptr(), rows, float(head_clamp), int(not want_x)
+        hent = ModconvPlugin._workspace(lib, ws_like, head_w, n, cout, rows, h, wd, 1, 0, True, arith)
+        e.w, e.rows, e.clamp, e.no_activation_output = head_w.data_ptr(), rows, float(head_clamp), int(not want_x)
         if head_bias is not None:
             head_bias = head_bias.contiguous()
             _require(head_bias.is_cuda and head_bias.dtype == torch.float32 and head_bias.numel() == rows, 'modconv2d_heads: head_bias must be float32 [rows] on GPU')
             e.bias = head_bias.data_ptr()
         e.workspace, e.workspace_bytes = hent[0].data_ptr(), hent[0].numel() * 4
         with _dev_guard(x.device):
-            rc = lib.ide3d_modconv2d_heads(ctypes.byref(p), ctypes.byref(e), _stream(x))
+            if skip is None:
+                rc = lib.ide3d_modconv2d_heads(ctypes.byref(p), ctypes.byref(e), _stream(x))
+            else:
+                rc = lib.ide3d_modconv2d_heads_skip(ctypes.byref(p), ctypes.byref(e), ctypes.byref(k), _stream(x))
         if rc == -2:
-            ModconvPlugin._heads_declined.add(shape_key)
+            if skip is None:
+                ModconvPlugin._heads_declined.add(shape_key)
+            elif 'IDE3D_MODCONV_NO_SKIP_FUSION' not in os.environ:
+                ModconvPlugin._heads_declined.add(skip_key)
             return None
         _check(rc, 'modconv2d_heads')
+        if skip is not None:
+            CALLS['modconv2d_heads_skip'] = CALLS.get('modconv2d_heads_skip', 0) + 1
         ModconvPlugin._ws.mark_packed(ent, (w,))
         return y, heads
 
diff --git a/ide-3d_amd/training/networks.py b/ide-3d_amd/training/networks.py
--- a/ide-3d_amd/training/networks.py
+++ b/ide-3d_amd/training/networks.py
@@ -546,7 +546,7 @@
     return y[:, :co], y[:, co:]
 
 
-def _conv1_dual_head(block, x, w1, w_shared, want_x, noise_mode='random', gain=1, input_noise=None, **unused):
+def _conv1_dual_head(block, x, w1, w_shared, want_x, noise_mode='random', gain=1, input_noise=None, skip=None, **unused):
     c1, tr, ts = block.conv1, block.torgb, block.toseg
     if not (use_hip_modconv and type(c1) is SynthesisLayer and c1.up == 1 and c1.padding == 1 and c1.weight.shape[2:] == (3, 3)
             and c1.activation in ('linear', 'lrelu') and tr.weight.shape[2] == 1 and tr.conv_clamp == ts.conv_clamp
@@ -573,9 +573,12 @@
     hbias = _cat_cached(tr.bias, ts.bias)
     hclamp = -1.0 if tr.conv_clamp is None else tr.conv_clamp
     xc = x.contiguous()
-    out = _modconv_plugin.modconv2d_heads(xc, c1.weight.contiguous(), styles.contiguous(), dcoefs, noise, 1.0, bias,
-                                          spec.cuda_idx, spec.def_alpha, act_gain, -1.0 if act_clamp is None else act_clamp,
-                                          wcat, hbias, hclamp, want_x=want_x)
+    args = (xc, c1.weight.contiguous(), styles.contiguous(), dcoefs, noise, 1.0, bias,
+            spec.cuda_idx, spec.def_alpha, act_gain, -1.0 if act_clamp is None else act_clamp, wcat, hbias, hclamp)
+    out = _modconv_plugin.modconv2d_heads(*args, want_x=want_x, skip=skip) if skip is not None else None
+    if out is not None:
+        return out
+    out = _modconv_plugin.modconv2d_heads(*args, want_x=want_x)
     if out is None:
         x = _modconv_bias_act(x, c1.weight, styles, True, noise, 1.0, bias, c1.activation, act_gain, act_clamp, dcoefs=dcoefs)
         return x, _dual_head(x, tr, ts, w_shared, wcat=wcat)
@@ -583,6 +586,8 @@
     co = tr.weight.shape[0]
     return x, (y[:, :co], y[:, co:])
 
+
+fuse_channels_last_skip = False
 
 _lowres_plugin = None
 
@@ -1134,6 +1139,17 @@
             return _upfirdn_plugin().upfirdn2d_ex(lo, f, 2, 2, 1, 1, 2, 1, 2, 1, False, 4.0, add=y)
         return cur.add_(y) if cur is not None else y
 
+    def _fusable_skip(self, x, img, seg):
+        if not (img is not None and seg is not None and img.ndim == 4 and seg.ndim == 4 and img.size(-1) * 2 == x.size(-1) and img.size(-2) * 2 == x.size(-2)
+                and seg.shape[2:] == img.shape[2:] and img.dtype == seg.dtype == torch.float32 and _inference_on_gpu(img, seg)
+                and self.resample_filter.shape == (4, 4) and self._filter_is_1331()):
+            return None
+        if getattr(self, 'skip_channels_last', False):
+            ok = fuse_channels_last_skip and img.shape[1] % 4 == 0 and seg.shape[1] % 4 == 0
+            return (img, seg, 'channels_last') if ok else None
+        joint = not self.is_last and not os.environ.get('IDE3D_NO_SKIP_MERGE') and _adjacent_views(img, seg) is not None
+        return (img, seg, 'joint' if joint else 'separate')
+
     def _filter_is_1331(self):
         ok = getattr(self, '_f1331', None)
         if ok is None:
@@ -1157,6 +1173,7 @@
                 fused_modconv = (not self.training) and (dtype == torch.float32 or int(ws.shape[0]) == 1)
 
         fused = fused_heads = None
+        skip_done = False
         if self.in_channels == 0:
             x = self.const.to(dtype=dtype, memory_format=memory_format)
             x = x.unsqueeze(0).expand(ws.shape[0], *x.size())
@@ -1174,9 +1191,11 @@
                 layer_kwargs['input_noise'] = block_noise[:, 1:2] if block_noise is not None else None
                 w1 = next(w_iter)
                 if (self.is_last or self.architecture == 'skip') and not disable_rgb and dtype == torch.float32:
-                    fused = _conv1_dual_head(self, x, w1, ws_list[self.num_conv], not x_unused, **layer_kwargs)
+                    fused = _conv1_dual_head(self, x, w1, ws_list[self.num_conv], not x_unused, skip=self._fusable_skip(x, img, seg), **layer_kwargs)
                 if fused is not None:
                     x, fused_heads = fused
+                    from torch_utils import hip_plugin
+                    skip_done = isinstance(fused_heads, hip_plugin.SkipImages)
                 else:
                     x = self.conv1(x, w1, fused_modconv=fused_modconv, **layer_kwargs)
 
@@ -1184,13 +1203,15 @@
         ref = x if x is not None else fused_heads[0]
         img_lo = seg_lo = None
         heads_follow = (self.is_last or self.architecture == 'skip') and not disable_rgb
-        if (heads_follow and _inference_on_gpu(ref, img, seg, w_shared, *_head_params(self.torgb, self.toseg)) and img is not None and seg is not None
+        if skip_done:
+            img, seg = fused_heads
+        elif (heads_follow and _inference_on_gpu(ref, img, seg, w_shared, *_head_params(self.torgb, self.toseg)) and img is not None and seg is not None
                 and img.size(-1) * 2 == ref.size(-1)):
             img_lo, seg_lo, img, seg = img, seg, None, None
         else:
             img = self._merge_skip(img, ref)
             seg = self._merge_skip(seg, ref)
-        if self.is_last or self.architecture == 'skip':
+        if (self.is_last or self.architecture == 'skip') and not skip_done:
             if disable_rgb:
                 img = seg = None
             else:
diff --git a/include/ide3d_hip.h b/include/ide3d_hip.h
--- a/include/ide3d_hip.h
+++ b/include/ide3d_hip.h
@@ -229,6 +229,18 @@
     int64_t      workspace_bytes;
 } ide3d_modconv_head_epilogue;
 int ide3d_modconv2d_heads(const ide3d_modconv_params* p, const ide3d_modconv_head_epilogue* heads, void* stream);
+
+typedef struct ide3d_modconv_skip_epilogue {
+    const float* lo[2];
+    int64_t      lo_stride[2][4];
+    float*       out[2];
+    int64_t      out_batch_stride[2];
+    int32_t      channels[2];
+    int32_t      channels_last;
+    int32_t      reserved;
+} ide3d_modconv_skip_epilogue;
+int ide3d_modconv2d_heads_skip(const ide3d_modconv_params* p, const ide3d_modconv_head_epilogue* heads, const ide3d_modconv_skip_epilogue* skip,
+                               void* stream);
 
 typedef struct ide3d_act_bwd_params {
     const float* dy;
```

After: 957.8 frames/s. About the same (-0.0%).
